# AgentMaker/PAPC

Hardware: AMD Instinct MI355X
Metric: point-clouds/sec (fwd+bwd) PointNet++SSG B=32 N=4096 (higher is better)
Workload: dtype f32

## Files before the change

### include/papc_hip.h

```cpp
#ifndef PAPC_HIP_H
#define PAPC_HIP_H

#include <stddef.h>
#include <stdint.h>

#ifdef __cplusplus
extern "C" {
#endif

#define PAPC_OK 0
#define PAPC_E_INVALID (-1)
#define PAPC_E_UNSUPPORTED (-2)
#define PAPC_E_LAUNCH (-3)

typedef void *papc_stream_t;

int papc_version(void);
#define PAPC_ABI_VERSION 8
int papc_abi_version(void);
int64_t papc_abi_sizeof(const char *struct_name);
const char *papc_last_error_string(void);


int papc_fps_f32(const float *xyz, int64_t sb, int64_t sn, int64_t sc, int B, int N, int npoint,
// ... 337 lines not shown
    const float *x; int32_t Cin, Cout;
    float *dy, *dw, *db, *dgamma, *dbeta; int32_t accumulate;
    int32_t phase;
} papc_head_bwd_job;
int papc_head_chain_fwd_f32(const papc_head_fc_layer *layers, int n_layers, int B, const int64_t *rng_state, int64_t *rng_bump,
                            const int64_t *labels, float *loss, float *dlogits, uint32_t *sync, papc_stream_t stream);
int papc_head_chain_bwd_f32(const papc_head_bwd_job *jobs, int n_jobs, int B, uint32_t *sync, papc_stream_t stream);

int papc_cloud_transform_f32(const float *x, int64_t sb, int64_t sn, int64_t sc, const float *T, int64_t ldt, int B, int N, int C, float *y,
                             papc_stream_t stream);
size_t papc_cloud_transform_bwd_workspace(int B, int N, int C);
int papc_cloud_transform_bwd_f32(const float *x, int64_t sb, int64_t sn, int64_t sc, const float *T, int64_t ldt, const float *dy, int B, int N, int C,
                                 float *dx, int64_t dsb, int64_t dsn, int64_t dsc, int accumulate, float *dT, void *workspace,
                                 size_t workspace_bytes, papc_stream_t stream);

int papc_cloud_concat_conv_parts(int B, int N);
int papc_cloud_concat_conv_f32(const float *x, int64_t ldx, const float *g, const float *w, const float *bias, int B, int N, int Cp, int Cg, int Cout,
                               float *y, float *cvec, float *stats_partial, papc_stream_t stream);
size_t papc_cloud_concat_conv_bwd_workspace(int B, int N, int Cp, int Cg, int Cout);
int papc_cloud_concat_conv_bwd_f32(const float *dz, const float *y, const float *mean, const float *invstd, const float *scale, const float *shift,
                                   const float *c1, const float *c2, const float *x, int64_t ldx, const float *g, const float *w, int B, int N, int Cp,
                                   int Cg, int Cout, float *dx, int64_t ldd, int accumulate, float *dw, float *dbias, float *dg, float *s_out,
                                   void *workspace, size_t workspace_bytes, papc_stream_t stream);

int papc_kdconv_ok(int dim, int Cin, int F);
int papc_kdconv_fwd_f32(const float *x, int64_t ldx, const int32_t *sel, int64_t sel_stride, const float *w, const float *bias, int B, int dim, int Cin,
                        int F, float *out, uint8_t *win, papc_stream_t stream);
size_t papc_kdconv_bwd_workspace(int B, int dim, int Cin, int F);
int papc_kdconv_bwd_f32(const float *gout, const float *out, const uint8_t *win, const float *x, int64_t ldx, const int32_t *sel, int64_t sel_stride,
                        const float *w, int B, int dim, int Cin, int F, float *dx, int64_t ldd, float *dw, float *dbias, int accumulate, void *workspace,
                        size_t workspace_bytes, papc_stream_t stream);

int papc_kdbn_ok(int dim, int Cin, int F);
size_t papc_kdbn_fwd_workspace(int B, int dim, int Cin, int F);
int papc_kdbn_fwd_f32(const float *x, int64_t ldx, const int32_t *sel, int64_t sel_stride, const float *w, const float *bias, const float *gamma,
                      const float *beta, float *running_mean, float *running_var, int B, int dim, int Cin, int F, float eps, float momentum, int training,
                      float *out, uint8_t *win, float *zhat, float *mean, float *tmat, float *stats, void *workspace, size_t workspace_bytes,
                      papc_stream_t stream);
size_t papc_kdbn_bwd_workspace(int B, int dim, int Cin, int F);
int papc_kdbn_bwd_f32(const float *gout, const float *out, const uint8_t *win, const float *zhat, const float *x, int64_t ldx, const int32_t *sel,
                      int64_t sel_stride, const float *w, const float *gamma, const float *mean, const float *tmat, const float *stats, int B, int dim,
                      int Cin, int F, int training, float *dx, int64_t ldd, float *dw, float *dbias, float *dgamma, float *dbeta, int accumulate,
                      void *workspace, size_t workspace_bytes, papc_stream_t stream);

int papc_voxconv_ok(int E);
int papc_voxconv_parts(int B, int E);
int papc_voxconv1_fwd_f32(const float *x, const float *w1, const float *b1, int B, int E, float *y1, float *stats_partial, papc_stream_t stream);
int papc_voxconv2_prep_f32(const float *w2, float *wk, float *wt, papc_stream_t stream);
int papc_voxconv2_pool_fwd_f32(const float *y1, const float *scale, const float *shift, const float *wk, const float *b2, int B, int E, float *out,
                               uint8_t *win, papc_stream_t stream);
int papc_voxconv2_bwd_dx_f32(const float *gout, const uint8_t *win, const float *wt, const float *y1, const float *mean, const float *invstd,
                             const float *scale, const float *shift, int B, int E, float *gp, float *dz, float *red_partial, papc_stream_t stream);
size_t papc_voxconv2_bwd_dw_workspace(int B, int E);
int papc_voxconv2_bwd_dw_f32(const float *gp, const uint8_t *win, const float *y1, const float *scale, const float *shift, int B, int E, float *dw2,
                             float *db2, int accumulate, void *workspace, size_t workspace_bytes, papc_stream_t stream);
size_t papc_voxconv1_bwd_dw_workspace(int B, int E);
int papc_voxconv1_bwd_dw_f32(const float *dz, const float *y1, const float *mean, const float *invstd, const float *scale, const float *c1, const float *c2,
                             const float *x, int B, int E, float *dw1, float *db1, int accumulate, void *workspace, size_t workspace_bytes,
                             papc_stream_t stream);
int papc_leaky_dropout_fwd_f32(const float *x, int64_t n, float slope, float drop_p, int64_t *rng_state, int tag, int bump, float *out, uint8_t *keep,
                               papc_stream_t stream);
int papc_leaky_dropout_bwd_f32(const float *gout, const float *x, const uint8_t *keep, int64_t n, float slope, float drop_p, float *dx,
                               papc_stream_t stream);
int papc_occupancy_grid_f32(const float *points, int B, int N, int E, float *grid, uint32_t *err, papc_stream_t stream);

size_t papc_nms_workspace(int N);
int papc_nms_f32(const float *dets, int N, float nms_overlap_thresh, int32_t *keep, int32_t *num_out, void *workspace,
                 size_t workspace_bytes, papc_stream_t stream);
int papc_rotate_nms_f32(const float *dets, int N, float nms_overlap_thresh, int32_t *keep, int32_t *num_out, void *workspace,
                        size_t workspace_bytes, papc_stream_t stream);
int papc_rotate_iou_f32(const float *boxes, const float *query_boxes, int N, int K, int criterion, float *iou, papc_stream_t stream);
int papc_rbbox_iou_f32(const float *box_corners, const float *qbox_corners, const float *standup_iou, float standup_thresh, int N, int K,
                       float *overlaps, papc_stream_t stream);
int papc_riou_f32(const float *rbboxes, const float *qrbboxes, float standup_thresh, int N, int K, float *overlaps, papc_stream_t stream);

int papc_lingather_parts(int64_t M);
int papc_mlp_compact_ok(int64_t M, int K, int n_layers, const int *couts);
int papc_compact_plan_f32(const int32_t *idx, int G, int K, int32_t *cnt8, int32_t *start, int32_t *rows, int32_t *cidx, int32_t *seg_grp,
                          float *wrow, float *coef, papc_stream_t stream);
int papc_compact_corr_parts(void);
int papc_bn_stats_corr_f32(const float *y, int C, const int32_t *start, const float *coef, int G, float *stats_rows, papc_stream_t stream);
int papc_bn_relu_max_seg_f32(const float *y, int C, const int32_t *start, const float *scale, const float *shift, int G, float *out,
                             int32_t *argmax, float *ysel, papc_stream_t stream);
int papc_lingather_fwd_f32(const float *P, const papc_group_src *grp, int B, const float *w, int ldw, int xcol0, const float *bias, int C,
                           float *y, float *stats_partial, papc_stream_t stream);
int papc_lingather_bwd_f32(const papc_bwd_dy *dy, const papc_group_src *grp, int B, int C, float *G, float *dwx_partial, papc_stream_t stream);
int papc_lingather_bwd_pp_ok(const papc_group_src *grp, int B, int C);
int papc_lingather_bwd_pp_f32(const papc_bwd_dy *dy, const papc_group_src *grp, int B, int C, const float *P, const float *w, int ldw, int xcol0,
                              const float *bias, float *G, float *dwx_partial, papc_stream_t stream);
int papc_lingather_list_parts(int64_t BN);
int papc_lingather_bwd_parts(const papc_group_src *grp, int B, int C);
int papc_lingather_bwd_lists_ok(const papc_group_src *grp, int C);
int papc_point_lists_f32(const papc_group_src *grp, int B, const int32_t *start, int32_t *prange, int32_t *prow, float *pmeta, float *pmom,
                         papc_stream_t stream);

int papc_mlp_bwd_dx_xyz_ok(int64_t M, int Cin, int Cout);
int papc_mlp_bwd_dx_xyz_f32(const papc_bwd_dy *dy, const float *wt, int64_t M, int Cin, int Cout, const float *xc, const float *wf,
                            float *partial, papc_stream_t stream);

int papc_bn_max_prep_f32(const float *gout, const float *ysel, const float *scale, const float *shift, const float *mean,
                         const float *invstd, const float *c1, const float *c2, const float *w, const float *bias, int64_t G, int Co,
                         int Ci, float *psel, float *wcat, float *hbias, float *e_out, float *q_out, papc_stream_t stream);
int papc_mlp_bwd_dx_max_f32(const float *psel, const int32_t *argmax, int K, const float *x, int64_t ldx, const float *bn_scale,
                            const float *bn_shift, const float *wcat, const float *hbias, int64_t M, int Cin, int Cout, float *dx,
                            const papc_bwd_red *next_red, papc_stream_t stream);

int papc_mlp_max_nostore_ok(int64_t M, int Cin, int Cout, int K);
int64_t papc_mlp_bwd_dw_max_ws_floats(int64_t M, int Cin, int Cout);
int papc_mlp_bwd_dw_max_f32(const float *psel, const int32_t *argmax, int K, const float *x, const float *bn_scale, const float *bn_shift,
                            const float *w, const float *e, const float *scale, const float *c1, int64_t M, int Cin, int Cout,
                            float *workspace, float *dw, int accumulate, papc_stream_t stream);

int papc_mlp_xyz_ok(int64_t M, int C1, int C2);
int papc_xyz_parts(int64_t M);
int papc_xyz_bwd_parts(int64_t M);
int papc_xyz_group_f32(const papc_group_src *grp, int B, float *xc, double *gram_partial, papc_stream_t stream);
int papc_xyz_gram_fold_f32(const double *gram_partial, int parts, double *gram, papc_stream_t stream);
int papc_xyz_l1_finalize_f32(const double *gram_partial, int parts, int64_t M, const float *w, int ldw, int xcol0, const float *bias,
                             const float *gamma, const float *beta, float eps, float momentum, int C, float *mean, float *invstd, float *scale,
                             float *shift, float *running_mean, float *running_var, float *wf, double *gram, papc_stream_t stream);
int papc_xyz_l1_bwd_f32(const float *dz, const float *xc, const float *wf, int64_t M, int C, float *partial, papc_stream_t stream);
int papc_xyz_l1_bwd_finalize_f32(const float *partial, int parts, int64_t M, int C, const double *gram, const float *w, int ldw, int xcol0,
                                 const float *bias, const float *mean, const float *invstd, const float *scale, float *dgamma, float *dbeta,
                                 float *dw, int accumulate, papc_stream_t stream);

size_t papc_pg_planes_bytes(int64_t R, int64_t K);

typedef struct papc_pg_wjob {
    const float *src;
    int64_t row_stride, col_stride;
    int R, K;
    void *planes;
} papc_pg_wjob;
int papc_pg_prep_weights_f32(const papc_pg_wjob *jobs, int count, papc_stream_t stream);

#define PAPC_PG_PLAIN 0
#define PAPC_PG_CONCAT 1
#define PAPC_PG_BNRELU 2
#define PAPC_PG_DY_DENSE 3
#define PAPC_PG_DY_MAX 4
typedef struct papc_pg_prep {
    int mode;
    int64_t M; int C;
    const float *x; int64_t ldx;
    const float *xyz; int64_t sb, sn, sc; const float *feats; int N, D, xyz_first;
    const float *dz;
    const float *gout, *ysel; const int32_t *argmax; int K;
    const float *stats; int parts;
    const float *gamma, *beta; float eps, momentum; float *running_mean, *running_var;
    float *mean, *invstd, *scale, *shift;
    const float *red; int red_parts;
    float *dgamma, *dbeta; int accumulate;
    void *planes, *planes_t;
} papc_pg_prep;
int papc_pg_prep_rows_f32(const papc_pg_prep *args, papc_stream_t stream);

#define PAPC_PG_STORE 0
#define PAPC_PG_FWD 1
#define PAPC_PG_FWD_GMAX 2
#define PAPC_PG_RED 3
typedef struct papc_pg_gemm {
    int epi;
    const void *a, *b;
    int R1, R2, K;
    float *c; int64_t ldc;
    int split; int64_t split_stride;
// ... 77 lines not shown
```

### papc_amd/_lib.py

```python
import ctypes
import os

_HERE = os.path.dirname(os.path.abspath(__file__))
LIB_PATH = os.environ.get("PAPC_LIB") or os.path.join(_HERE, "libpapc_hip.so")

ABI_VERSION = 8

c_p = ctypes.c_void_p
c_i = ctypes.c_int
c_l = ctypes.c_int64
c_f = ctypes.c_float


class PapcError(RuntimeError):
    pass


class GroupSrc(ctypes.Structure):
    _fields_ = [("xyz", c_p), ("sb", c_l), ("sn", c_l), ("sc", c_l), ("new_xyz", c_p), ("feats", c_p),
                ("idx", c_p), ("N", c_i), ("S", c_i), ("K", c_i), ("D", c_i), ("xyz_first", c_i),
                ("cidx", c_p), ("seg_grp", c_p), ("rows_dev", c_p), ("wstat", c_p), ("plists", c_p)]


class PointLists(ctypes.Structure):
    _fields_ = [("prange", c_p), ("prow", c_p), ("pmeta", c_p), ("compact", c_i), ("pmom", c_p)]


class BwdDy(ctypes.Structure):
    _fields_ = [("dz_mode", c_i), ("dz", c_p), ("gout", c_p), ("argmax", c_p), ("K", c_i), ("y", c_p),
                ("mean", c_p), ("invstd", c_p), ("scale", c_p), ("shift", c_p), ("c1", c_p), ("c2", c_p),
                ("wrow", c_p), ("seg_grp", c_p), ("rows_dev", c_p), ("psel", c_p)]

    def set_bn(self, y, cst, c12):
        self.y = ptr(y)
        self.mean, self.invstd, self.scale, self.shift = cst_ptrs(cst)
        self.c1, self.c2 = c12.data_ptr(), c12.data_ptr() + 4 * c12.stride(0)


class GroupMax(ctypes.Structure):
    _fields_ = [("gmax", c_p), ("gmin", c_p), ("amax", c_p), ("amin", c_p), ("K", c_i), ("sign_src", c_p)]


class BwdRed(ctypes.Structure):
    _fields_ = [("y", c_p), ("mean", c_p), ("invstd", c_p), ("scale", c_p), ("shift", c_p), ("red_partial", c_p), ("store_masked", c_i)]


class CopyJob(ctypes.Structure):
    _fields_ = [("src", ctypes.c_void_p), ("dst", ctypes.c_void_p), ("B", ctypes.c_int32), ("R", ctypes.c_int32), ("C", ctypes.c_int32),
                ("sb", ctypes.c_int64), ("sr", ctypes.c_int64), ("sc", ctypes.c_int64), ("db", ctypes.c_int64), ("dr", ctypes.c_int64),
                ("dc", ctypes.c_int64)]


class ReduceJob(ctypes.Structure):
    _fields_ = [("partial", c_p), ("n_chunks", ctypes.c_int32), ("accumulate", ctypes.c_int32), ("ld", c_l), ("n1", c_l), ("n2", c_l),
                ("out1", c_p), ("out2", c_p)]


class ScatterDst(ctypes.Structure):
    _fields_ = [("grad_feats", c_p), ("idx", c_p), ("N", c_i), ("S", c_i), ("K", c_i), ("D", c_i), ("col0", c_i)]


SIGNATURES = {
    "papc_version": (c_i, []),
    "papc_abi_version": (c_i, []),
    "papc_abi_sizeof": (c_l, [ctypes.c_char_p]),
    "papc_last_error_string": (ctypes.c_char_p, []),
    "papc_fps_f32": (c_i, [c_p, c_l, c_l, c_l, c_i, c_i, c_i, c_p, c_f, c_p, c_p, c_p]),
    "papc_ball_query_f32": (c_i, [c_p, c_l, c_l, c_l, c_p, c_i, c_i, c_i, c_i, c_p, c_p, c_p, c_i, c_p]),
    "papc_square_distance_f32": (c_i, [c_p, c_p, c_i, c_i, c_i, c_p, c_p]),
    "papc_index_points_f32": (c_i, [c_p, c_p, c_i, c_i, c_i, c_i, c_i, c_p, c_p]),
    "papc_index_points_bwd_f32": (c_i, [c_p, c_p, c_i, c_i, c_i, c_i, c_i, c_p, c_p]),
    "papc_group_points_f32": (c_i, [c_p, c_l, c_l, c_l, c_p, c_p, c_p, c_i, c_i, c_i, c_i, c_i, c_i, c_p, c_p]),
    "papc_group_points_bwd_f32": (c_i, [c_p, c_p, c_i, c_i, c_i, c_i, c_i, c_i, c_p, c_p, c_p, c_p]),
    "papc_three_nn_f32": (c_i, [c_p, c_l, c_l, c_l, c_p, c_l, c_l, c_l, c_i, c_i, c_i, c_p, c_p, c_p, c_p]),
    "papc_three_interpolate_f32": (c_i, [c_p, c_p, c_p, c_i, c_i, c_i, c_i, c_p, c_p]),
    "papc_three_interpolate_bwd_f32": (c_i, [c_p, c_p, c_p, c_i, c_i, c_i, c_i, c_p, c_p]),
    "papc_three_interpolate_bwd_first3_f32": (c_i, [c_p, c_p, c_i, c_i, c_i, c_i, c_p, c_p]),
    "papc_mlp_gemm_parts": (c_i, [c_l]),
    "papc_mlp_gemm_gmax_ok": (c_i, [c_l, c_i, c_i]),
    "papc_mlp_gemm_f32": (c_i, [c_i, c_p, c_l, c_p, c_p, c_p, c_p, c_p, c_l, c_i, c_i, c_p, c_p, c_p, c_p]),
    "papc_mlp_gemm_rows_f32": (c_i, [c_i, c_p, c_l, c_p, c_p, c_p, c_p, c_p, c_l, c_i, c_i, c_p, c_p, c_p, c_p, c_p]),
    "papc_mlp_gemm_rows_w_f32": (c_i, [c_i, c_p, c_l, c_p, c_p, c_p, c_p, c_p, c_l, c_i, c_i, c_p, c_p, c_p, c_p, c_p, c_p]),
    "papc_sa_mlp_plan": (c_i, [c_p, c_p, c_p]),
    "papc_sa_mlp_fwd": (c_i, [c_p, c_p, c_p]),
    "papc_sa_mlp_bwd": (c_i, [c_p, c_p, c_p, c_p]),
    "papc_pfn_workspace": (c_i, [c_p, c_p, c_p]),
    "papc_pfn_fwd": (c_i, [c_p, c_p, c_p]),
    "papc_pfn_bwd": (c_i, [c_p, c_p, c_p, c_p, c_p, c_p, c_i, c_p]),
    "papc_compact_plan_f32": (c_i, [c_p, c_i, c_i, c_p, c_p, c_p, c_p, c_p, c_p, c_p, c_p]),
    "papc_compact_corr_parts": (c_i, []),
    "papc_mlp_compact_ok": (c_i, [c_l, c_i, c_i, c_p]),
    "papc_bn_stats_corr_f32": (c_i, [c_p, c_i, c_p, c_p, c_i, c_p, c_p]),
    "papc_bn_relu_max_seg_f32": (c_i, [c_p, c_i, c_p, c_p, c_p, c_i, c_p, c_p, c_p, c_p]),
    "papc_bn_select_max_f32": (c_i, [c_p, c_p, c_p, c_p, c_p, c_p, c_l, c_i, c_p, c_p, c_p]),
    "papc_bn_finalize_f32": (c_i, [c_p, c_i, c_l, c_i, c_p, c_p, c_f, c_f, c_p, c_p, c_p, c_p, c_p, c_p, c_p]),
    "papc_bn_relu_max_f32": (c_i, [c_p, c_p, c_p, c_l, c_i, c_i, c_p, c_p, c_p]),
    "papc_bn_relu_f32": (c_i, [c_p, c_p, c_p, c_l, c_i, c_p, c_p]),
    "papc_bn_bwd_reduce_max_f32": (c_i, [c_p, c_p, c_i, c_p, c_p, c_p, c_p, c_l, c_i, c_i, c_p, c_p, c_p]),
    "papc_bn_bwd_reduce_f32": (c_i, [c_i, c_p, c_p, c_p, c_i, c_p, c_p, c_p, c_p, c_p, c_l, c_i, c_i, c_p, c_p]),
    "papc_bn_bwd_finalize_f32": (c_i, [c_p, c_i, c_l, c_i, c_p, c_p, c_p, c_p, c_i, c_p]),
    "papc_bn_eval_consts_f32": (c_i, [c_p, c_p, c_p, c_p, c_f, c_i, c_p, c_p, c_p, c_p, c_p]),
    "papc_group_max_bwd_f32": (c_i, [c_p, c_p, c_l, c_i, c_i, c_p, c_p]),
    "papc_mlp_bwd_dx_f32": (c_i, [c_p, c_p, c_l, c_i, c_i, c_p, c_p, c_p, c_p]),
    "papc_mlp_bwd_dw_f32": (c_i, [c_p, c_i, c_p, c_l, c_p, c_p, c_p, c_l, c_i, c_i, c_i, c_p, c_p, c_l, c_p]),
    "papc_reduce_partials2_f32": (c_i, [c_p, c_i, c_l, c_l, c_p, c_l, c_p, c_i, c_p]),
    "papc_reduce_partials_batch_f32": (c_i, [c_p, c_i, c_p]),
    "papc_fold_jobs_f32": (c_i, [c_p, c_i, c_p]),
    "papc_mlp_bwd_dw_chunk_hint": (c_i, [c_l, c_i, c_i, c_i, c_i, c_i]),
    "papc_reduce_partials_f32": (c_i, [c_p, c_i, c_l, c_p, c_i, c_p]),
    "papc_pfn_decorate_f32": (c_i, [c_p, c_p, c_p, c_i, c_i, c_f, c_f, c_f, c_f, c_i, c_p, c_p]),
    "papc_pfn_decorate_nf_f32": (c_i, [c_p, c_i, c_p, c_p, c_i, c_i, c_f, c_f, c_f, c_f, c_i, c_p, c_p]),
    "papc_pfn_stats_f32": (c_i, [c_p, c_p, c_p, c_i, c_i, c_f, c_f, c_f, c_f, c_p, c_i, c_p, c_p, c_p]),
    "papc_pfn_apply_f32": (c_i, [c_p, c_p, c_p, c_i, c_i, c_f, c_f, c_f, c_f, c_p, c_i, c_p, c_p, c_p, c_p, c_p]),
    "papc_pfn_num_blocks": (c_i, [c_i]),
    "papc_pfn_bwd_reduce_f32": (c_i, [c_p, c_p, c_p, c_i, c_i, c_f, c_f, c_f, c_f, c_p, c_i, c_p, c_p, c_p, c_p, c_p, c_p, c_p, c_p]),
    "papc_pfn_bwd_dw_f32": (c_i, [c_p, c_p, c_p, c_i, c_i, c_f, c_f, c_f, c_f, c_p, c_i, c_p, c_p, c_p, c_p, c_p, c_p, c_p, c_p, c_p, c_p]),
    "papc_pfn_gram_blocks": (c_i, [c_i]),
    "papc_pfn_gram_f32": (c_i, [c_p, c_p, c_p, c_i, c_i, c_f, c_f, c_f, c_f, c_p, c_p]),
    "papc_pfn_gram_finalize_f32": (c_i, [c_p, c_i, c_l, c_p, c_i, c_p, c_p, c_f, c_f, c_p, c_p, c_p, c_p, c_p, c_p, c_p, c_p]),
    "papc_pfn_bwd_sparse_f32": (c_i, [c_p, c_p, c_p, c_i, c_i, c_f, c_f, c_f, c_f, c_p, c_i, c_p, c_p, c_p, c_p, c_p, c_p, c_p, c_p]),
    "papc_pfn_bwd_finalize_f32": (c_i, [c_p, c_l, c_p, c_i, c_p, c_p, c_p, c_p, c_p, c_p, c_p, c_i, c_p]),
    "papc_points_to_voxel_workspace": (ctypes.c_size_t, [c_i]),
    "papc_points_to_voxel_f32": (c_i, [c_p, c_i, c_i, c_p, c_p, c_i, c_i, c_i, c_p, c_p, c_p, c_p, c_p, ctypes.c_size_t, c_p]),
    "papc_pillar_scatter_f32": (c_i, [c_p, c_p, c_i, c_i, c_i, c_i, c_i, c_p, c_p, c_p]),
    "papc_pillar_scatter_bwd_f32": (c_i, [c_p, c_p, c_p, c_i, c_i, c_i, c_i, c_i, c_p, c_p]),
    "papc_head_fc_f32": (c_i, [c_p, c_p, c_p, c_p, c_p, c_i, c_i, c_i, c_i, c_f, c_f, c_p, c_p, c_p, c_f, c_p, c_i, c_p, c_p, c_p, c_p,
                               c_p, c_p, c_p]),
    "papc_head_bwd_f32": (c_i, [c_p, c_p, c_i, c_p, c_p, c_p, c_p, c_p, c_f, c_i, c_p, c_i, c_i, c_i, c_p, c_p, c_p, c_p, c_p, c_i, c_p]),
    "papc_softmax_xent_f32": (c_i, [c_p, c_p, c_i, c_i, c_p, c_p, c_p]),
    "papc_head_chain_fwd_f32": (c_i, [c_p, c_i, c_i, c_p, c_p, c_p, c_p, c_p, c_p, c_p]),
    "papc_head_chain_bwd_f32": (c_i, [c_p, c_i, c_i, c_p, c_p]),
    "papc_cloud_transform_f32": (c_i, [c_p, c_l, c_l, c_l, c_p, c_l, c_i, c_i, c_i, c_p, c_p]),
    "papc_cloud_transform_bwd_workspace": (ctypes.c_size_t, [c_i, c_i, c_i]),
    "papc_cloud_transform_bwd_f32": (c_i, [c_p, c_l, c_l, c_l, c_p, c_l, c_p, c_i, c_i, c_i, c_p, c_l, c_l, c_l, c_i, c_p, c_p, ctypes.c_size_t, c_p]),
    "papc_cloud_concat_conv_parts": (c_i, [c_i, c_i]),
    "papc_cloud_concat_conv_f32": (c_i, [c_p, c_l, c_p, c_p, c_p, c_i, c_i, c_i, c_i, c_i, c_p, c_p, c_p, c_p]),
    "papc_cloud_concat_conv_bwd_workspace": (ctypes.c_size_t, [c_i, c_i, c_i, c_i, c_i]),
    "papc_cloud_concat_conv_bwd_f32": (c_i, [c_p, c_p, c_p, c_p, c_p, c_p, c_p, c_p, c_p, c_l, c_p, c_p, c_i, c_i, c_i, c_i, c_i, c_p, c_l, c_i, c_p, c_p,
                                             c_p, c_p, c_p, ctypes.c_size_t, c_p]),
    "papc_kdconv_ok": (c_i, [c_i, c_i, c_i]),
    "papc_kdconv_fwd_f32": (c_i, [c_p, c_l, c_p, c_l, c_p, c_p, c_i, c_i, c_i, c_i, c_p, c_p, c_p]),
    "papc_kdconv_bwd_workspace": (ctypes.c_size_t, [c_i, c_i, c_i, c_i]),
    "papc_kdconv_bwd_f32": (c_i, [c_p, c_p, c_p, c_p, c_l, c_p, c_l, c_p, c_i, c_i, c_i, c_i, c_p, c_l, c_p, c_p, c_i, c_p, ctypes.c_size_t, c_p]),
    "papc_kdbn_ok": (c_i, [c_i, c_i, c_i]),
    "papc_kdbn_fwd_workspace": (ctypes.c_size_t, [c_i, c_i, c_i, c_i]),
    "papc_kdbn_fwd_f32": (c_i, [c_p, c_l, c_p, c_l, c_p, c_p, c_p, c_p, c_p, c_p, c_i, c_i, c_i, c_i, c_f, c_f, c_i, c_p, c_p, c_p, c_p, c_p, c_p, c_p,
                                ctypes.c_size_t, c_p]),
    "papc_kdbn_bwd_workspace": (ctypes.c_size_t, [c_i, c_i, c_i, c_i]),
    "papc_kdbn_bwd_f32": (c_i, [c_p, c_p, c_p, c_p, c_p, c_l, c_p, c_l, c_p, c_p, c_p, c_p, c_p, c_i, c_i, c_i, c_i, c_i, c_p, c_l, c_p, c_p, c_p, c_p, c_i,
                                c_p, ctypes.c_size_t, c_p]),
    "papc_voxconv_ok": (c_i, [c_i]),
    "papc_voxconv_parts": (c_i, [c_i, c_i]),
    "papc_voxconv1_fwd_f32": (c_i, [c_p, c_p, c_p, c_i, c_i, c_p, c_p, c_p]),
    "papc_voxconv2_prep_f32": (c_i, [c_p, c_p, c_p, c_p]),
    "papc_voxconv2_pool_fwd_f32": (c_i, [c_p, c_p, c_p, c_p, c_p, c_i, c_i, c_p, c_p, c_p]),
    "papc_voxconv2_bwd_dx_f32": (c_i, [c_p] * 8 + [c_i, c_i, c_p, c_p, c_p, c_p]),
    "papc_voxconv2_bwd_dw_workspace": (ctypes.c_size_t, [c_i, c_i]),
    "papc_voxconv2_bwd_dw_f32": (c_i, [c_p, c_p, c_p, c_p, c_p, c_i, c_i, c_p, c_p, c_i, c_p, ctypes.c_size_t, c_p]),
    "papc_voxconv1_bwd_dw_workspace": (ctypes.c_size_t, [c_i, c_i]),
    "papc_voxconv1_bwd_dw_f32": (c_i, [c_p] * 8 + [c_i, c_i, c_p, c_p, c_i, c_p, ctypes.c_size_t, c_p]),
    "papc_leaky_dropout_fwd_f32": (c_i, [c_p, c_l, c_f, c_f, c_p, c_i, c_i, c_p, c_p, c_p]),
    "papc_leaky_dropout_bwd_f32": (c_i, [c_p, c_p, c_p, c_l, c_f, c_f, c_p, c_p]),
    "papc_occupancy_grid_f32": (c_i, [c_p, c_i, c_i, c_i, c_p, c_p, c_p]),
    "papc_nms_workspace": (ctypes.c_size_t, [c_i]),
    "papc_nms_f32": (c_i, [c_p, c_i, c_f, c_p, c_p, c_p, ctypes.c_size_t, c_p]),
    "papc_lingather_parts": (c_i, [c_l]),
    "papc_lingather_fwd_f32": (c_i, [c_p, c_p, c_i, c_p, c_i, c_i, c_p, c_i, c_p, c_p, c_p]),
    "papc_lingather_bwd_f32": (c_i, [c_p, c_p, c_i, c_i, c_p, c_p, c_p]),
    "papc_lingather_bwd_pp_f32": (c_i, [c_p, c_p, c_i, c_i, c_p, c_p, c_i, c_i, c_p, c_p, c_p, c_p]),
    "papc_lingather_list_parts": (c_i, [c_l]),
    "papc_lingather_bwd_parts": (c_i, [c_p, c_i, c_i]),
    "papc_lingather_bwd_lists_ok": (c_i, [c_p, c_i]),
    "papc_point_lists_f32": (c_i, [c_p, c_i, c_p, c_p, c_p, c_p, c_p, c_p]),
    "papc_lingather_bwd_pp_ok": (c_i, [c_p, c_i, c_i]),
    "papc_bn_max_prep_f32": (c_i, [c_p] * 10 + [c_l, c_i, c_i] + [c_p] * 6),
    "papc_mlp_max_nostore_ok": (c_i, [c_l, c_i, c_i, c_i]),
# ... 146 lines not shown
```

### papc_amd/csrc/bn_ops.hip

```cpp
#include "common.h"

namespace papc {

template <int V> struct Vec;
template <> struct Vec<4> {
    float4 v;
    __device__ static Vec load(const float *p) { Vec r; r.v = *reinterpret_cast<const float4 *>(p); return r; }
    __device__ void store(float *p) const { *reinterpret_cast<float4 *>(p) = v; }
    __device__ float &operator[](int i) { return (&v.x)[i]; }
    __device__ float operator[](int i) const { return (&v.x)[i]; }
};
template <> struct Vec<1> {
    float v;
    __device__ static Vec load(const float *p) { Vec r; r.v = *p; return r; }
    __device__ void store(float *p) const { *p = v; }
    __device__ float &operator[](int) { return v; }
    __device__ float operator[](int) const { return v; }
};

template <int D>
__device__ __forceinline__ void sum_partial_rows_d(const float *__restrict__ part, int n_tiles, int C, int c, int tl, double &s1, double &s2)
{
    for (int t0 = tl; t0 < n_tiles; t0 += 64 * D) {
        float a[D], b[D];
#pragma unroll
        for (int j = 0; j < D; ++j) {
            const int t = t0 + 64 * j;
            const int64_t o = (int64_t)(t < n_tiles ? t : t0) * 2 * C + c;
            a[j] = part[o];
            b[j] = part[o + C];
        }
#pragma unroll
        for (int j = 0; j < D; ++j) {
            if (t0 + 64 * j < n_tiles) { s1 += (double)a[j]; s2 += (double)b[j]; }
        }
    }
}
__device__ __forceinline__ void sum_partial_rows(const float *__restrict__ part, int n_tiles, int C, int c, int tl, double &s1, double &s2)
{
    if (n_tiles > 512) sum_partial_rows_d<16>(part, n_tiles, C, c, tl, s1, s2);
    else sum_partial_rows_d<8>(part, n_tiles, C, c, tl, s1, s2);
}

__device__ __forceinline__ double lane_get(double v, int l)
{
    const int lo = __builtin_amdgcn_readlane(__double2loint(v), l), hi = __builtin_amdgcn_readlane(__double2hiint(v), l);
    return __hiloint2double(hi, lo);
}
__device__ __forceinline__ void fold_part_lanes(double &s1, double &s2)
{
    s1 += __shfl_xor(s1, 1); s2 += __shfl_xor(s2, 1);
    s1 += __shfl_xor(s1, 2); s2 += __shfl_xor(s2, 2);
    double t1 = 0.0, t2 = 0.0;
#pragma unroll
    for (int w = 0; w < 16; ++w) { t1 += lane_get(s1, 4 * w); t2 += lane_get(s2, 4 * w); }
    s1 = t1; s2 = t2;
}

__global__ __launch_bounds__(64) void bn_finalize_kernel(const float *__restrict__ part, int n_tiles, int64_t M, int C,
                                                        const float *__restrict__ gamma, const float *__restrict__ beta,
                                                        float eps, float momentum, float *mean, float *invstd, float *scale,
                                                        float *shift, float *rmean, float *rvar)
{
    const int c = blockIdx.x, tl = threadIdx.x;
    const float gam = gamma ? gamma[c] : 1.f, bet = beta ? beta[c] : 0.f;
    const float rm0 = rmean ? rmean[c] : 0.f, rv0 = rvar ? rvar[c] : 0.f;
    double s1 = 0.0, s2 = 0.0;
    sum_partial_rows(part, n_tiles, C, c, tl, s1, s2);
    fold_part_lanes(s1, s2);
    if (tl == 0) {
        const double mu = s1 / (double)M;
        double var = s2 / (double)M - mu * mu;
        if (var < 0.0) var = 0.0;
        const double is = 1.0 / sqrt(var + (double)eps);
        const double sc = (double)gam * is;
        mean[c] = (float)mu;
        invstd[c] = (float)is;
        scale[c] = (float)sc;
        shift[c] = (float)((double)bet - mu * sc);
        if (rmean) rmean[c] = momentum * rm0 + (1.f - momentum) * (float)mu;
        if (rvar) rvar[c] = momentum * rv0 + (1.f - momentum) * (float)var;
    }
}

template <int V>
__global__ __launch_bounds__(256) void bn_relu_max_kernel(const float *__restrict__ y, const float *__restrict__ scale,
                                                          const float *__restrict__ shift, int64_t G, int K, int C,
                                                          float *__restrict__ out, int32_t *__restrict__ argmax)
{
    const int CV = C / V;
    const int64_t total = G * CV;
    for (int64_t e = (int64_t)blockIdx.x * blockDim.x + threadIdx.x; e < total; e += (int64_t)gridDim.x * blockDim.x) {
        const int64_t g = e / CV;
        const int c = (int)(e - g * CV) * V;
        const Vec<V> sc = Vec<V>::load(scale + c), sh = Vec<V>::load(shift + c);
        Vec<V> best;
        int bi[V];
#pragma unroll
        for (int i = 0; i < V; ++i) { best[i] = -1.0f; bi[i] = 0; }
        const float *yp = y + (g * K) * (int64_t)C + c;
        for (int k = 0; k < K; ++k) {
            const Vec<V> v = Vec<V>::load(yp + (int64_t)k * C);
#pragma unroll
            for (int i = 0; i < V; ++i) {
                const float z = relu_np(fmaf(sc[i], v[i], sh[i]));
                if (z > best[i] || z != z) { best[i] = z; bi[i] = k; }
            }
        }
        best.store(out + g * C + c);
        if (argmax) {
#pragma unroll
            for (int i = 0; i < V; ++i) argmax[g * C + c + i] = bi[i];
        }
    }
}

__global__ __launch_bounds__(256) void bn_select_max_kernel(float *__restrict__ gmax, const float *__restrict__ gmin,
                                                            const int32_t *__restrict__ amax, const int32_t *__restrict__ amin,
                                                            const float *__restrict__ scale, const float *__restrict__ shift,
                                                            int64_t total, int C, float *__restrict__ out, int32_t *__restrict__ argmax)
{
    for (int64_t e = (int64_t)blockIdx.x * blockDim.x + threadIdx.x; e < total; e += (int64_t)gridDim.x * blockDim.x) {
        const int c = (int)(e % C);
        const float sc = scale[c], sh = shift[c];
        const bool up = sc >= 0.f;
        const float sel = up ? gmax[e] : gmin[e];
        out[e] = relu_np(fmaf(sc, sel, sh));
        gmax[e] = sel;
        if (argmax) argmax[e] = up ? amax[e] : amin[e];
    }
}

template <int V>
__global__ __launch_bounds__(256) void bn_relu_kernel(const float *__restrict__ y, const float *__restrict__ scale,
                                                      const float *__restrict__ shift, int64_t M, int C, float *__restrict__ z)
{
    const int CV = C / V;
    const int64_t total = M * CV;
    for (int64_t e = (int64_t)blockIdx.x * blockDim.x + threadIdx.x; e < total; e += (int64_t)gridDim.x * blockDim.x) {
        const int c = (int)(e % CV) * V;
        const Vec<V> sc = Vec<V>::load(scale + c), sh = Vec<V>::load(shift + c);
        Vec<V> v = Vec<V>::load(y + e * V);
#pragma unroll
        for (int i = 0; i < V; ++i) v[i] = fmaxf(fmaf(sc[i], v[i], sh[i]), 0.f);
        v.store(z + e * V);
    }
}

template <int V, bool MAXMODE>
__global__ __launch_bounds__(256) void bn_bwd_reduce_kernel(const float *__restrict__ dz, const float *__restrict__ gout,
                                                            const int32_t *__restrict__ argmax, int K,
                                                            const float *__restrict__ y, const float *__restrict__ mean,
                                                            const float *__restrict__ invstd, const float *__restrict__ scale,
                                                            const float *__restrict__ shift, int64_t M, int C,
                                                            float *__restrict__ part, float *__restrict__ psel_out = nullptr)
{
    __shared__ float red[2][256 * 4];
    const int CV = C / V;
    const int CG = CV < 256 ? CV : 256;
    const int RL = 256 / CG;
    const int cgi = threadIdx.x % CG, rl = threadIdx.x / CG;
    const int64_t units = MAXMODE ? M / K : M;
    const int64_t per = (units + gridDim.x - 1) / gridDim.x;
    const int64_t u0 = (int64_t)blockIdx.x * per, u1 = min(units, u0 + per);

// ... 296 lines not shown

__global__ __launch_bounds__(256) void bn_max_psel_kernel(const float *__restrict__ gout, const float *__restrict__ ysel,
                                                          const float *__restrict__ scale, const float *__restrict__ shift, int64_t total,
                                                          int C, float *__restrict__ psel)
{
    for (int64_t e = (int64_t)blockIdx.x * blockDim.x + threadIdx.x; e < total; e += (int64_t)gridDim.x * blockDim.x) {
        const int c = (int)(e % C);
        const float sc = scale[c];
        psel[e] = fmaf(sc, ysel[e], shift[c]) > 0.f ? sc * gout[e] : 0.f;
    }
}

__global__ __launch_bounds__(256) void bn_max_wcat_kernel(const float *__restrict__ w, const float *__restrict__ bias,
                                                          const float *__restrict__ scale, const float *__restrict__ mean,
                                                          const float *__restrict__ invstd, const float *__restrict__ c1,
                                                          const float *__restrict__ c2, int Co, int Ci, float *__restrict__ wcat,
                                                          float *__restrict__ hbias, float *__restrict__ e_out, float *__restrict__ q_out)
{
    extern __shared__ float sm[];
    float *ewn = sm;
    double *red = reinterpret_cast<double *>(sm + ((Co + 1) & ~1));
    const int n = blockIdx.x, tid = threadIdx.x;
    double hacc = 0.0;
    for (int c = tid; c < Co; c += 256) {
        const float s = scale[c];
        const float e = s * c2[c] * invstd[c];
        const float q = e * (mean[c] - (bias ? bias[c] : 0.f)) - s * c1[c];
        const float wv = w[(int64_t)c * Ci + n];
        ewn[c] = e * wv;
        hacc += (double)q * (double)wv;
        wcat[(int64_t)n * (Co + Ci) + c] = wv;
        if (n == 0) { e_out[c] = e; q_out[c] = q; }
    }
    red[tid] = hacc;
    __syncthreads();
    for (int st = 128; st > 0; st >>= 1) {
        if (tid < st) red[tid] += red[tid + st];
        __syncthreads();
    }
    if (tid == 0) hbias[n] = (float)red[0];
    for (int j = tid; j < Ci; j += 256) {
        double g = 0.0;
        for (int c = 0; c < Co; ++c) g += (double)ewn[c] * (double)w[(int64_t)c * Ci + j];
        wcat[(int64_t)n * (Co + Ci) + Co + j] = (float)(-g);
    }
}

struct TransposeBatch {
    const float *src[8];
    float *dst[8];
    int rows[8], cols[8];
    int ld[8], copy[8];
};

__global__ __launch_bounds__(256) void transpose_batch_kernel(TransposeBatch t)
{
    __shared__ float tile[32][33];
    const int m = blockIdx.y;
    const int rows = t.rows[m], cols = t.cols[m];
    const int tiles_c = (cols + 31) >> 5, tiles = ((rows + 31) >> 5) * tiles_c;
    const float *__restrict__ src = t.src[m];
    float *__restrict__ dst = t.dst[m];
    const int tx = threadIdx.x & 31, ty = threadIdx.x >> 5;
    for (int tl = blockIdx.x; tl < tiles; tl += gridDim.x) {
        const int r0 = (tl / tiles_c) * 32, c0 = (tl % tiles_c) * 32;
#pragma unroll
        for (int i = 0; i < 4; ++i) {
            const int r = r0 + ty + 8 * i, c = c0 + tx;
            const float v = (r < rows && c < cols) ? src[(int64_t)r * t.ld[m] + c] : 0.f;
            tile[ty + 8 * i][tx] = v;
            if (t.copy[m] && r < rows && c < cols) dst[(int64_t)r * cols + c] = v;
        }
        if (t.copy[m]) continue;
        __syncthreads();
#pragma unroll
        for (int i = 0; i < 4; ++i) {
            const int c = c0 + ty + 8 * i, r = r0 + tx;
            if (r < rows && c < cols) dst[(int64_t)c * rows + r] = tile[tx][ty + 8 * i];
        }
        __syncthreads();
    }
}

}


using namespace papc;

extern "C" {

int papc_bn_finalize_f32(const float *stats_partial, int n_tiles, int64_t M, int C, const float *gamma,
                         const float *beta, float eps, float momentum, float *mean, float *invstd,
                         float *scale, float *shift, float *running_mean, float *running_var,
                         papc_stream_t stream)
{
    PAPC_REQUIRE(stats_partial && mean && invstd && scale && shift, PAPC_E_INVALID, "papc_bn_finalize_f32: null pointer");
    PAPC_REQUIRE(n_tiles >= 1 && M >= 1 && C >= 1, PAPC_E_INVALID, "papc_bn_finalize_f32: bad sizes");
    hipStream_t st = as_stream(stream);
    ProfScope prof(PAPC_K_MISC, st);
    hipLaunchKernelGGL(bn_finalize_kernel, dim3((unsigned)C), dim3(64), 0, st, stats_partial, n_tiles, M, C, gamma,
                       beta, eps, momentum, mean, invstd, scale, shift, running_mean, running_var);
    return check_launch("papc_bn_finalize_f32");
}

int papc_bn_relu_max_f32(const float *y, const float *scale, const float *shift, int64_t G, int K, int C,
                         float *out, int32_t *argmax, papc_stream_t stream)
{
    PAPC_REQUIRE(y && scale && shift && out, PAPC_E_INVALID, "papc_bn_relu_max_f32: null pointer");
    PAPC_REQUIRE(G >= 1 && K >= 1 && C >= 1, PAPC_E_INVALID, "papc_bn_relu_max_f32: bad sizes");
    hipStream_t st = as_stream(stream);
    ProfScope prof(PAPC_K_BN_RELU_MAX, st);
    const bool v4 = (C % 4 == 0) && aligned16(y) && aligned16(scale) && aligned16(shift) && aligned16(out);
    if (v4 && K >= 256 && G * (C / 4) < 65536 && G <= 65535) {
        hipLaunchKernelGGL(bn_relu_max_split_kernel, dim3((unsigned)G, (unsigned)cdiv(C, 256)), dim3(1024), 0, st, y, scale, shift, G, K, C, out, argmax);
        return check_launch("papc_bn_relu_max_f32");
    }
    if (v4) hipLaunchKernelGGL(bn_relu_max_kernel<4>, dim3(ew_grid(G * (C / 4))), dim3(256), 0, st, y, scale, shift, G, K, C, out, argmax);
    else hipLaunchKernelGGL(bn_relu_max_kernel<1>, dim3(ew_grid(G * C)), dim3(256), 0, st, y, scale, shift, G, K, C, out, argmax);
    return check_launch("papc_bn_relu_max_f32");
}

int papc_bn_select_max_f32(float *gmax, const float *gmin, const int32_t *amax, const int32_t *amin,
                           const float *scale, const float *shift, int64_t G, int C, float *out, int32_t *argmax,
                           papc_stream_t stream)
{
    PAPC_REQUIRE(gmax && gmin && amax && amin && scale && shift && out, PAPC_E_INVALID, "papc_bn_select_max_f32: null pointer");
    PAPC_REQUIRE(G >= 1 && C >= 1, PAPC_E_INVALID, "papc_bn_select_max_f32: bad sizes");
    hipStream_t st = as_stream(stream);
    ProfScope prof(PAPC_K_BN_RELU_MAX, st);
    hipLaunchKernelGGL(bn_select_max_kernel, dim3(ew_grid(G * C)), dim3(256), 0, st, gmax, gmin, amax, amin, scale, shift, G * C, C, out, argmax);
    return check_launch("papc_bn_select_max_f32");
}

int papc_bn_relu_f32(const float *y, const float *scale, const float *shift, int64_t M, int C, float *z, papc_stream_t stream)
{
    PAPC_REQUIRE(y && scale && shift && z, PAPC_E_INVALID, "papc_bn_relu_f32: null pointer");
    PAPC_REQUIRE(M >= 1 && C >= 1, PAPC_E_INVALID, "papc_bn_relu_f32: bad sizes");
    hipStream_t st = as_stream(stream);
    ProfScope prof(PAPC_K_MISC, st);
    const bool v4 = (C % 4 == 0) && aligned16(y) && aligned16(scale) && aligned16(shift) && aligned16(z);
    if (v4) hipLaunchKernelGGL(bn_relu_kernel<4>, dim3(ew_grid(M * (C / 4))), dim3(256), 0, st, y, scale, shift, M, C, z);
    else hipLaunchKernelGGL(bn_relu_kernel<1>, dim3(ew_grid(M * C)), dim3(256), 0, st, y, scale, shift, M, C, z);
    return check_launch("papc_bn_relu_f32");
}

int papc_bn_bwd_reduce_f32(int dz_mode, const float *dz, const float *gout, const int32_t *argmax, int K,
                           const float *y, const float *mean, const float *invstd, const float *scale,
                           const float *shift, int64_t M, int C, int n_parts, float *red_partial, papc_stream_t stream)
{
    PAPC_REQUIRE(mean && invstd && scale && shift && red_partial, PAPC_E_INVALID, "papc_bn_bwd_reduce_f32: null pointer");
    PAPC_REQUIRE(y || (dz_mode != PAPC_DZ_DENSE && dz), PAPC_E_INVALID, "papc_bn_bwd_reduce_f32: y may be NULL only in MAX mode with dz = ysel");
    PAPC_REQUIRE(M >= 1 && C >= 1 && n_parts >= 1, PAPC_E_INVALID, "papc_bn_bwd_reduce_f32: bad sizes");
    hipStream_t st = as_stream(stream);
    ProfScope prof(PAPC_K_BWD_REDUCE, st);
    if (dz_mode == PAPC_DZ_DENSE) {
        PAPC_REQUIRE(dz, PAPC_E_INVALID, "papc_bn_bwd_reduce_f32: DENSE needs dz");
        const bool v4 = (C % 4 == 0) && aligned16(dz) && aligned16(y) && aligned16(mean) && aligned16(invstd) && aligned16(scale) && aligned16(shift);
        if (v4) hipLaunchKernelGGL((bn_bwd_reduce_kernel<4, false>), dim3(n_parts), dim3(256), 0, st, dz, gout, argmax, K, y, mean, invstd, scale, shift, M, C, red_partial);
        else hipLaunchKernelGGL((bn_bwd_reduce_kernel<1, false>), dim3(n_parts), dim3(256), 0, st, dz, gout, argmax, K, y, mean, invstd, scale, shift, M, C, red_partial);
    } else {
        PAPC_REQUIRE(gout && argmax && K >= 1 && M % K == 0, PAPC_E_INVALID, "papc_bn_bwd_reduce_f32: MAX needs gout/argmax and K | M");
        const bool v4 = (C % 4 == 0) && aligned16(gout) && (!dz || aligned16(dz)) && aligned16(mean) && aligned16(invstd) && aligned16(scale) && aligned16(shift);
        if (v4) hipLaunchKernelGGL((bn_bwd_reduce_kernel<4, true>), dim3(n_parts), dim3(256), 0, st, dz, gout, argmax, K, y, mean, invstd, scale, shift, M, C, red_partial);
        else hipLaunchKernelGGL((bn_bwd_reduce_kernel<1, true>), dim3(n_parts), dim3(256), 0, st, dz, gout, argmax, K, y, mean, invstd, scale, shift, M, C, red_partial);
    }
    return check_launch("papc_bn_bwd_reduce_f32");
// ... 224 lines not shown
```

### papc_amd/csrc/capi.hip

```cpp
#include <stdarg.h>
#include <string.h>

#include <mutex>
#include <vector>

#include "common.h"

#define GEMM_PARTS_DEFAULT 768

namespace papc {

static thread_local char g_err[512] = "";

void set_error(const char *fmt, ...)
{
    va_list ap;
    va_start(ap, fmt);
    vsnprintf(g_err, sizeof(g_err), fmt, ap);
    va_end(ap);
}

int check_launch(const char *what)
{
    hipError_t e = hipGetLastError();
    if (e != hipSuccess) {
        set_error("%s: %s", what, hipGetErrorString(e));
        return PAPC_E_LAUNCH;
    }
    return PAPC_OK;
}

struct KnobDef { const char *name; int def, lo, hi; };
static const KnobDef g_knob_defs[KNOB_COUNT] = {
    {"PAPC_LG_PARTS", 2048, 1, 8192},
    {"PAPC_DW_F32", 0, 0, 1},
    {"PAPC_DW_DBG", 0, 0, 1},
    {"PAPC_DW_XYZ", 1, 0, 1},
    {"PAPC_PARTS", GEMM_PARTS_DEFAULT, 1, 1024},
    {"PAPC_GEMM_F32", 0, 0, 1},
    {"PAPC_GEMM_WAVES", 0, 0, 8},
    {"PAPC_MAXCAT_WAVES", 8, 4, 8},
    {"PAPC_GEMM_WS", 0, 0, 3},
    {"PAPC_GEMM_OCC", 0, 0, 1},
    {"PAPC_GEMM_DBG", 0, 0, 1},
    {"PAPC_GEMM_KB", 0, 0, 2},
    {"PAPC_GEMM_MINWG", 192, 1, 4096},
    {"PAPC_GEMM_TL", 0, 0, 1},
    {"PAPC_FPS_THREADS", 0, 0, 1024},
    {"PAPC_FPS_THREADS_SMALL", 0, 0, 1024},
    {"PAPC_STREAM", 1, 0, 1},
    {"PAPC_STREAM_MINTILES", 2048, 1, 1 << 30},
    {"PAPC_STREAM_CK", 0, 0, 8},
    {"PAPC_STREAM_ASM", 1, 0, 1},
    {"PAPC_PFN_MFMA", 1, 0, 1},
    {"PAPC_DW_RS64", 1, 0, 1},
    {"PAPC_DW_ROWS", 1, 0, 1},
    {"PAPC_DW_ROWS_BLOCKS", 4, 1, 16},
    {"PAPC_DW_ROWSX", 1, 0, 1},
    {"PAPC_PG_DBG", 0, 0, 15},
    {"PAPC_PG_NB", 0, 0, 2},
    {"PAPC_PG_NS", 0, 0, 3},
    {"PAPC_STREAM_MAXCAT", 1, 0, 1},
    {"PAPC_MAX_NOSTORE", 1, 0, 1},
    {"PAPC_PFN_FUSED_TAILS", 1, 0, 1},
    {"PAPC_STREAM_NW12", 1, 0, 1},
    {"PAPC_LG_LISTS", 1, 0, 1},
    {"PAPC_FOLD_WAVES", 16, 8, 16},
    {"PAPC_LGL_VARIANT", 0, 0, 3},
    {"PAPC_LG_PP", 1, 0, 1},
    {"PAPC_PG_GROUP", 1, 0, 1},
    {"PAPC_PG_PIPE", 1, 0, 1},
};
static int g_knobs[KNOB_COUNT];
static int knob_parse(int id, const char *e)
{
    const KnobDef &d = g_knob_defs[id];
    if (!e || !*e) return d.def;
    const int v = atoi(e);
    return (v < d.lo || v > d.hi) ? d.def : v;
}
static const bool g_knobs_loaded = [] {
    for (int i = 0; i < KNOB_COUNT; ++i) g_knobs[i] = knob_parse(i, getenv(g_knob_defs[i].name));
    return true;
}();
int knob(int id) { return g_knobs[id]; }

struct ProfState {
    std::mutex mu;
    unsigned mask = 0;
    std::vector<std::pair<hipEvent_t, hipEvent_t>> pending[PAPC_K_COUNT];
    std::vector<hipEvent_t> pool;
    double total_ms[PAPC_K_COUNT] = {0};
    int64_t launches[PAPC_K_COUNT] = {0};
};
static ProfState g_prof;

static hipEvent_t prof_get_event()
{
    if (!g_prof.pool.empty()) {
        hipEvent_t e = g_prof.pool.back();
        g_prof.pool.pop_back();
        return e;
    }
    hipEvent_t e;
    if (hipEventCreate(&e) != hipSuccess) return nullptr;
    return e;
}

ProfScope::ProfScope(int k, hipStream_t s) : kernel(k), stream(s), on(false), e0(nullptr)
{
    if (!(g_prof.mask & (1u << k))) return;
    std::lock_guard<std::mutex> lk(g_prof.mu);
    e0 = prof_get_event();
    if (!e0) return;
    on = hipEventRecord(e0, stream) == hipSuccess;
}

ProfScope::~ProfScope()
{
    if (!on) return;
    std::lock_guard<std::mutex> lk(g_prof.mu);
    hipEvent_t e1 = prof_get_event();
    if (!e1) return;
    if (hipEventRecord(e1, stream) == hipSuccess) g_prof.pending[kernel].push_back({e0, e1});
}

static void prof_drain(int k)
{
    for (auto &pr : g_prof.pending[k]) {
        float ms = 0.f;
        if (hipEventSynchronize(pr.second) == hipSuccess && hipEventElapsedTime(&ms, pr.first, pr.second) == hipSuccess) {
            g_prof.total_ms[k] += ms;
            g_prof.launches[k] += 1;
        }
        g_prof.pool.push_back(pr.first);
        g_prof.pool.push_back(pr.second);
    }
    g_prof.pending[k].clear();
}

}

extern "C" {

int papc_version(void) { return 600;  }

int papc_abi_version(void) { return PAPC_ABI_VERSION; }

int64_t papc_abi_sizeof(const char *struct_name)
{
    if (!struct_name) return -1;
#define PAPC_SIZEOF(T) if (strcmp(struct_name, #T) == 0) return (int64_t)sizeof(T);
    PAPC_SIZEOF(papc_group_src)
    PAPC_SIZEOF(papc_point_lists)
// ... 81 lines not shown
```

### papc_amd/csrc/common.h

```cpp
#pragma once
#include <hip/hip_runtime.h>
#include <stdint.h>
#include <stdio.h>
#include <stdlib.h>
#include <string.h>
#include <algorithm>

#include "papc_hip.h"

namespace papc {

void set_error(const char *fmt, ...);
int check_launch(const char *what);

#define PAPC_REQUIRE(cond, code, ...)      \
    do {                                   \
        if (!(cond)) {                     \
            papc::set_error(__VA_ARGS__);  \
            return (code);                 \
        }                                  \
    } while (0)

enum Knob {
    KNOB_LG_PARTS, KNOB_DW_F32, KNOB_DW_DBG, KNOB_DW_XYZ, KNOB_PARTS, KNOB_GEMM_F32, KNOB_GEMM_WAVES, KNOB_MAXCAT_WAVES,
    KNOB_GEMM_WS, KNOB_GEMM_OCC, KNOB_GEMM_DBG, KNOB_GEMM_KB, KNOB_GEMM_MINWG, KNOB_GEMM_TL, KNOB_FPS_THREADS,
    KNOB_FPS_THREADS_SMALL, KNOB_STREAM, KNOB_STREAM_MINTILES, KNOB_STREAM_CK, KNOB_STREAM_ASM, KNOB_PFN_MFMA, KNOB_DW_RS64, KNOB_DW_ROWS, KNOB_DW_ROWS_BLOCKS, KNOB_DW_ROWSX, KNOB_PG_DBG, KNOB_PG_NB, KNOB_PG_NS, KNOB_STREAM_MAXCAT, KNOB_MAX_NOSTORE, KNOB_PFN_FUSED_TAILS, KNOB_STREAM_NW12, KNOB_LG_LISTS, KNOB_FOLD_WAVES, KNOB_LGL_VARIANT, KNOB_LG_PP, KNOB_PG_GROUP, KNOB_PG_PIPE, KNOB_COUNT
};
int knob(int id);

struct ProfScope {
    int kernel;
    hipStream_t stream;
    bool on;
    hipEvent_t e0;
    ProfScope(int kernel, hipStream_t stream);
    ~ProfScope();
};

static inline hipStream_t as_stream(papc_stream_t s) { return reinterpret_cast<hipStream_t>(s); }

static inline int64_t cdiv(int64_t a, int64_t b) { return (a + b - 1) / b; }
static inline bool aligned16(const void *p) { return (reinterpret_cast<uintptr_t>(p) & 15) == 0; }

#define PAPC_DPP(v, ctrl, rmask) __builtin_amdgcn_update_dpp((int)(v), (int)(v), (ctrl), (rmask), 0xF, false)

__device__ __forceinline__ float wave_sum_f32_to_lane63(float v)
{
    float t;
    t = __int_as_float(PAPC_DPP(__float_as_int(v), 0xB1, 0xF));  v += t;
    t = __int_as_float(PAPC_DPP(__float_as_int(v), 0x4E, 0xF));  v += t;
    t = __int_as_float(PAPC_DPP(__float_as_int(v), 0x124, 0xF)); v += t;
    t = __int_as_float(PAPC_DPP(__float_as_int(v), 0x128, 0xF)); v += t;
    t = __int_as_float(__builtin_amdgcn_update_dpp(0, __float_as_int(v), 0x142, 0xA, 0xF, false)); v += t;
    t = __int_as_float(__builtin_amdgcn_update_dpp(0, __float_as_int(v), 0x143, 0xC, 0xF, false)); v += t;
    return v;
}

__device__ __forceinline__ float half_sum_f32(float v)
{
    float t;
    t = __int_as_float(PAPC_DPP(__float_as_int(v), 0xB1, 0xF));  v += t;
    t = __int_as_float(PAPC_DPP(__float_as_int(v), 0x4E, 0xF));  v += t;
    t = __int_as_float(PAPC_DPP(__float_as_int(v), 0x124, 0xF)); v += t;
    t = __int_as_float(PAPC_DPP(__float_as_int(v), 0x128, 0xF)); v += t;
    t = __int_as_float(__builtin_amdgcn_update_dpp(0, __float_as_int(v), 0x142, 0xA, 0xF, false)); v += t;
    return v;
}

__device__ __forceinline__ float readlane63_f32(float v)
{
    return __int_as_float(__builtin_amdgcn_readlane(__float_as_int(v), 63));
}


#define PAPC_DPPF(v, ctrl, rmask) __int_as_float(__builtin_amdgcn_update_dpp(__float_as_int(v), __float_as_int(v), (ctrl), (rmask), 0xF, false))
#define PAPC_DPPU(v, ctrl, rmask) ((unsigned)__builtin_amdgcn_update_dpp((int)(v), (int)(v), (ctrl), (rmask), 0xF, false))

__device__ __forceinline__ float row_max_f32(float v)
{
    v = fmaxf(v, PAPC_DPPF(v, 0xB1, 0xF));
    v = fmaxf(v, PAPC_DPPF(v, 0x4E, 0xF));
    v = fmaxf(v, PAPC_DPPF(v, 0x124, 0xF));
    v = fmaxf(v, PAPC_DPPF(v, 0x128, 0xF));
    return v;
}
__device__ __forceinline__ unsigned row_min_u32(unsigned v)
{
    unsigned t;
    t = PAPC_DPPU(v, 0xB1, 0xF);  v = t < v ? t : v;
    t = PAPC_DPPU(v, 0x4E, 0xF);  v = t < v ? t : v;
    t = PAPC_DPPU(v, 0x124, 0xF); v = t < v ? t : v;
    t = PAPC_DPPU(v, 0x128, 0xF); v = t < v ? t : v;
    return v;
}
__device__ __forceinline__ float wave_max_f32_to_lane63(float v)
{
    v = row_max_f32(v);
    v = fmaxf(v, PAPC_DPPF(v, 0x142, 0xA));
    v = fmaxf(v, PAPC_DPPF(v, 0x143, 0xC));
    return v;
}
__device__ __forceinline__ unsigned wave_min_u32_to_lane63(unsigned v)
{
    unsigned t;
    v = row_min_u32(v);
    t = PAPC_DPPU(v, 0x142, 0xA); v = t < v ? t : v;
    t = PAPC_DPPU(v, 0x143, 0xC); v = t < v ? t : v;
    return v;
}
// ... 47 lines not shown
```

### papc_amd/csrc/compact.hip

```cpp
#include "common.h"

namespace papc {

__global__ __launch_bounds__(256) void compact_count_kernel(const int32_t *__restrict__ idx, int G, int K, int32_t *__restrict__ cnt8)
{
    const int g = blockIdx.x * 4 + (threadIdx.x >> 6), lane = threadIdx.x & 63;
    if (g >= G) return;
    const int32_t *row = idx + (int64_t)g * K;
    const int32_t first = row[0];
    int n = 0;
    for (int k = lane; k < K; k += 64) n += (k > 0 && row[k] != first) ? 1 : 0;
#pragma unroll
    for (int o = 32; o > 0; o >>= 1) n += __shfl_xor(n, o);
    if (lane == 0) cnt8[g] = (n + 1 + 7) & ~7;
}

__global__ __launch_bounds__(1024) void compact_scan_kernel(const int32_t *__restrict__ cnt8, int G, int32_t *__restrict__ start,
                                                            int32_t *__restrict__ rows)
{
    __shared__ int part[1024];
    const int tid = threadIdx.x;
    const int per = (G + 1023) / 1024;
    const int g0 = tid * per, g1 = min(G, g0 + per);
    int s = 0;
// ... 60 lines not shown
                }
#pragma unroll
                for (int u = 0; u < U; ++u) {
                    s1.x = fmaf(cf[u], v[u].x, s1.x); s1.y = fmaf(cf[u], v[u].y, s1.y); s1.z = fmaf(cf[u], v[u].z, s1.z); s1.w = fmaf(cf[u], v[u].w, s1.w);
                    s2.x = fmaf(cf[u] * v[u].x, v[u].x, s2.x); s2.y = fmaf(cf[u] * v[u].y, v[u].y, s2.y);
                    s2.z = fmaf(cf[u] * v[u].z, v[u].z, s2.z); s2.w = fmaf(cf[u] * v[u].w, v[u].w, s2.w);
                }
            }
        }
        red[0][threadIdx.x] = s1; red[1][threadIdx.x] = s2;
        __syncthreads();
        const int cqn = CQ < 256 ? CQ : 256;
        if ((int)threadIdx.x < cqn && c0 + (int)threadIdx.x < CQ) {
            float4 t1 = make_float4(0.f, 0.f, 0.f, 0.f), t2 = t1;
            for (int l = 0; l < RL; ++l) {
                const float4 a = red[0][l * cqn + threadIdx.x], b = red[1][l * cqn + threadIdx.x];
                t1.x += a.x; t1.y += a.y; t1.z += a.z; t1.w += a.w;
                t2.x += b.x; t2.y += b.y; t2.z += b.z; t2.w += b.w;
            }
            *reinterpret_cast<float4 *>(out + ((int64_t)r * 2 + 0) * C + 4 * (c0 + threadIdx.x)) = t1;
            *reinterpret_cast<float4 *>(out + ((int64_t)r * 2 + 1) * C + 4 * (c0 + threadIdx.x)) = t2;
        }
        __syncthreads();
    }
}

__global__ __launch_bounds__(256) void seg_max_kernel(const float *__restrict__ y, int C, const int32_t *__restrict__ start,
                                                      const float *__restrict__ scale, const float *__restrict__ shift, int G,
                                                      float *__restrict__ out, int32_t *__restrict__ argmax, float *__restrict__ ysel)
{
    const int CQ = C >> 2;
    const int64_t e = (int64_t)blockIdx.x * 256 + threadIdx.x;
    if (e >= (int64_t)G * CQ) return;
    const int g = (int)(e / CQ), c = (int)(e - (int64_t)g * CQ) * 4;
    const int r0 = start[g], r1 = start[g + 1];
    const float4 sc = *reinterpret_cast<const float4 *>(scale + c), sh = *reinterpret_cast<const float4 *>(shift + c);
    const float s4[4] = {sc.x, sc.y, sc.z, sc.w}, h4[4] = {sh.x, sh.y, sh.z, sh.w};
    int flip[4];
#pragma unroll
    for (int i = 0; i < 4; ++i) flip[i] = s4[i] >= 0.f ? 0 : (int)0x80000000u;
    float mx[4] = {-INFINITY, -INFINITY, -INFINITY, -INFINITY};
    int ix[4] = {r0, r0, r0, r0};
    const float *p = y + (int64_t)r0 * C + c;
    int r = r0;
    for (; r + 4 <= r1; r += 4) {
        float4 v[4];
#pragma unroll
        for (int u = 0; u < 4; ++u) v[u] = *reinterpret_cast<const float4 *>(p + (int64_t)u * C);
#pragma unroll
        for (int u = 0; u < 4; ++u) {
            const float a[4] = {v[u].x, v[u].y, v[u].z, v[u].w};
#pragma unroll
            for (int i = 0; i < 4; ++i) {
                const float k = __int_as_float(__float_as_int(a[i]) ^ flip[i]);
                if (k > mx[i]) { mx[i] = k; ix[i] = r + u; }
            }
        }
        p += (int64_t)4 * C;
    }
    for (; r < r1; ++r) {
        const float4 v = *reinterpret_cast<const float4 *>(p);
        const float a[4] = {v.x, v.y, v.z, v.w};
#pragma unroll
        for (int i = 0; i < 4; ++i) {
            const float k = __int_as_float(__float_as_int(a[i]) ^ flip[i]);
            if (k > mx[i]) { mx[i] = k; ix[i] = r; }
        }
        p += C;
    }
    float o[4], ys[4];
    int am[4];
#pragma unroll
    for (int i = 0; i < 4; ++i) {
        ys[i] = __int_as_float(__float_as_int(mx[i]) ^ flip[i]);
        am[i] = ix[i];
        o[i] = relu_np(fmaf(s4[i], ys[i], h4[i]));
    }
    const int64_t q = (int64_t)g * C + c;
    *reinterpret_cast<float4 *>(out + q) = make_float4(o[0], o[1], o[2], o[3]);
    *reinterpret_cast<int4 *>(argmax + q) = make_int4(am[0], am[1], am[2], am[3]);
    *reinterpret_cast<float4 *>(ysel + q) = make_float4(ys[0], ys[1], ys[2], ys[3]);
}

}

using namespace papc;

extern "C" {

int papc_compact_plan_f32(const int32_t *idx, int G, int K, int32_t *cnt8, int32_t *start, int32_t *rows, int32_t *cidx, int32_t *seg_grp,
                          float *wrow, float *coef, papc_stream_t stream)
{
    PAPC_REQUIRE(idx && cnt8 && start && rows && cidx && seg_grp && wrow && coef, PAPC_E_INVALID, "papc_compact_plan_f32: null pointer");
    PAPC_REQUIRE(G >= 1 && K >= 8 && K % 8 == 0, PAPC_E_UNSUPPORTED, "papc_compact_plan_f32: G=%d, nsample=%d must be a multiple of 8", G, K);
    PAPC_REQUIRE((int64_t)G * K < (1ll << 31), PAPC_E_UNSUPPORTED, "papc_compact_plan_f32: >= 2^31 rows");
    hipStream_t st = as_stream(stream);
    ProfScope prof(PAPC_K_GROUP, st);
    const unsigned nb = (unsigned)cdiv(G, 4);
    hipLaunchKernelGGL(compact_count_kernel, dim3(nb), dim3(256), 0, st, idx, G, K, cnt8);
    hipLaunchKernelGGL(compact_scan_kernel, dim3(1), dim3(1024), 0, st, cnt8, G, start, rows);
    hipLaunchKernelGGL(compact_fill_kernel, dim3(nb), dim3(256), 0, st, idx, G, K, start, rows, cidx, seg_grp, wrow, coef);
    return check_launch("papc_compact_plan_f32");
}

int papc_compact_corr_parts(void) { return 64; }

int papc_bn_stats_corr_f32(const float *y, int C, const int32_t *start, const float *coef, int G, float *stats_rows, papc_stream_t stream)
{
    PAPC_REQUIRE(y && start && coef && stats_rows, PAPC_E_INVALID, "papc_bn_stats_corr_f32: null pointer");
    PAPC_REQUIRE(G >= 1 && C >= 4 && C % 4 == 0 && aligned16(y) && aligned16(stats_rows), PAPC_E_INVALID, "papc_bn_stats_corr_f32: C %% 4 == 0 and 16-byte aligned rows");
    hipStream_t st = as_stream(stream);
    ProfScope prof(PAPC_K_MISC, st);
    hipLaunchKernelGGL(bn_stats_corr_kernel, dim3((unsigned)papc_compact_corr_parts()), dim3(256), 0, st, y, C, start, coef, G, stats_rows);
    return check_launch("papc_bn_stats_corr_f32");
}

int papc_bn_relu_max_seg_f32(const float *y, int C, const int32_t *start, const float *scale, const float *shift, int G, float *out,
                             int32_t *argmax, float *ysel, papc_stream_t stream)
{
    PAPC_REQUIRE(y && start && scale && shift && out && argmax && ysel, PAPC_E_INVALID, "papc_bn_relu_max_seg_f32: null pointer");
    PAPC_REQUIRE(G >= 1 && C >= 4 && C % 4 == 0, PAPC_E_UNSUPPORTED, "papc_bn_relu_max_seg_f32: C=%d must be a multiple of 4", C);
    PAPC_REQUIRE(aligned16(y) && aligned16(scale) && aligned16(shift) && aligned16(out) && aligned16(argmax) && aligned16(ysel), PAPC_E_INVALID,
                 "papc_bn_relu_max_seg_f32: 16-byte alignment");
    hipStream_t st = as_stream(stream);
    ProfScope prof(PAPC_K_BN_RELU_MAX, st);
    hipLaunchKernelGGL(seg_max_kernel, dim3((unsigned)cdiv((int64_t)G * (C / 4), 256)), dim3(256), 0, st, y, C, start, scale, shift, G, out, argmax, ysel);
    return check_launch("papc_bn_relu_max_seg_f32");
}

}
```

### papc_amd/csrc/mlp_gemm.h

```cpp
#pragma once
#include "mlp_loaders.h"

namespace papc {

enum { EPI_STORE = 0, EPI_SCATTER = 1, EPI_STORE_RED = 2, EPI_STORE_GMAX = 3, EPI_GMAX = 4, EPI_XYZ_RED = 5 };

struct RedSrc {
    const float *y; const float *mean, *invstd, *scale, *shift;
    int masked;
};

struct ScatterDst {
    float *gf; const int32_t *idx; int N, S, K, D;
    FastDiv divSK, divK;
};

struct GmaxDst {
    float *gmax, *gmin; int32_t *amax, *amin; int K;
    const float *sgn;
};

struct GemmArgs {
    ASrc a;
    const float *w; int64_t ldw;
    int wmap;
    int nmap;
    const float *bias;
    int64_t M; int Kin; int Nout;
    float *y; int64_t ldy;
    float *stats;
    int parts;
    ScatterDst sc;
    RedSrc rd;
    GmaxDst gm;
    const int32_t *rows_dev;
    const float *wstat;
    unsigned long long *dbg;
    int tl;
};

constexpr int GEMM_MAX_PARTS = 768;

int stream_gemm_try(const GemmArgs &p, int amode, int epi, bool vec, hipStream_t st);

}
```

### papc_amd/csrc/mlp_gemm.hip

```cpp
#include "mlp_gemm.h"
#include <mutex>
#include <unordered_map>

namespace papc {

constexpr int LDT = 36;
constexpr int BK = 32;

template <bool VEC, bool WMAP, bool NMAP>
__device__ __forceinline__ float4 fetch_w4(const GemmArgs &p, int n, int k)
{
    const int nn = n < p.Nout ? n : 0;
    const int nrow = NMAP ? gk(p.a.g, nn) : nn;
    const float *wr = p.w + (int64_t)nrow * p.ldw;
    float4 v;
    if (WMAP) {
        v.x = wr[k < p.Kin ? gk(p.a.g, k) : 0];
        v.y = wr[k + 1 < p.Kin ? gk(p.a.g, k + 1) : 0];
        v.z = wr[k + 2 < p.Kin ? gk(p.a.g, k + 2) : 0];
        v.w = wr[k + 3 < p.Kin ? gk(p.a.g, k + 3) : 0];
    } else if (VEC) {
        v = ld4(wr + (k < p.Kin ? k : 0));
    } else {
        v.x = wr[k < p.Kin ? k : 0];
// ... 805 lines not shown
    g.idx = s->idx; g.N = s->N; g.S = s->S; g.K = s->K; g.D = s->D; g.xyz_first = s->xyz_first;
    g.divK = make_fastdiv((uint32_t)s->K);
    g.divS = make_fastdiv((uint32_t)s->S);
}

void fill_dy(DySrc &d, const papc_bwd_dy *s)
{
    d.dz = s->dz; d.gout = s->gout; d.argmax = s->argmax; d.K = s->K > 0 ? s->K : 1; d.y = s->y; d.mean = s->mean;
    d.invstd = s->invstd; d.scale = s->scale; d.shift = s->shift; d.c1 = s->c1; d.c2 = s->c2;
    d.divK = make_fastdiv((uint32_t)d.K);
    d.C = 0;
    d.wrow = s->wrow; d.seg_grp = s->seg_grp; d.rows_dev = s->rows_dev; d.psel = s->psel;
}

int check_dy(const papc_bwd_dy *dy, int64_t M, int C, bool *vec, const char *who)
{
    PAPC_REQUIRE(dy && dy->y && dy->mean && dy->invstd && dy->scale && dy->shift && dy->c1 && dy->c2, PAPC_E_INVALID,
                 "%s: null pointer in dy", who);
    const bool cst = aligned16(dy->mean) && aligned16(dy->invstd) && aligned16(dy->scale) && aligned16(dy->shift) &&
                     aligned16(dy->c1) && aligned16(dy->c2);
    if (dy->dz_mode == PAPC_DZ_DENSE) {
        PAPC_REQUIRE(dy->dz, PAPC_E_INVALID, "%s: DENSE needs dz", who);
        *vec = cst && aligned16(dy->dz) && aligned16(dy->y) && (C % 4 == 0);
    } else if (dy->dz_mode == PAPC_DZ_MAX) {
        PAPC_REQUIRE(dy->gout && dy->argmax && dy->K >= 1 && M % dy->K == 0, PAPC_E_INVALID, "%s: MAX needs gout/argmax and K | M", who);
        *vec = cst && aligned16(dy->gout) && aligned16(dy->argmax) && aligned16(dy->y) && (C % 4 == 0);
    } else {
        set_error("%s: bad dz_mode %d", who, dy->dz_mode);
        return PAPC_E_INVALID;
    }
    return PAPC_OK;
}

int fill_asrc(ASrc &a, int a_mode, const float *x, int64_t ldx, const papc_group_src *grp, const float *sc,
              const float *sh, int Cin, const char *who)
{
    memset(&a, 0, sizeof(a));
    if (a_mode == A_PLAIN || a_mode == A_BNRELU) {
        PAPC_REQUIRE(x && ldx >= Cin, PAPC_E_INVALID, "%s: x null or ldx < Cin", who);
        PAPC_REQUIRE(a_mode == A_PLAIN || (sc && sh), PAPC_E_INVALID, "%s: BNRELU needs bn_scale/bn_shift", who);
        a.x = x; a.ldx = ldx; a.sc = sc; a.sh = sh;
        a.vec = aligned16(x) && (ldx % 4 == 0) && (Cin % 4 == 0) && (a_mode == A_PLAIN || (aligned16(sc) && aligned16(sh)));
    } else if (a_mode == A_XYZ) {
        PAPC_REQUIRE(x && ldx == 4 && sc, PAPC_E_INVALID, "%s: XYZ needs xc [M, 4] (ldx = 4) and the folded first layer wf [Cin, 4] as bn_scale", who);
        a.x = x; a.ldx = 4; a.sc = sc; a.sh = nullptr;
        a.vec = aligned16(x) && aligned16(sc) && Cin % 4 == 0;
    } else if (a_mode == A_GROUP) {
        PAPC_REQUIRE(grp && grp->xyz && grp->new_xyz, PAPC_E_INVALID, "%s: GROUP needs grp->xyz/new_xyz", who);
        PAPC_REQUIRE(grp->D == 0 || grp->feats, PAPC_E_INVALID, "%s: GROUP D=%d but feats null", who, grp->D);
        PAPC_REQUIRE(Cin == grp->D + 3, PAPC_E_INVALID, "%s: GROUP Cin=%d != D+3=%d", who, Cin, grp->D + 3);
        PAPC_REQUIRE(grp->N >= 1 && grp->S >= 1 && grp->K >= 1, PAPC_E_INVALID, "%s: GROUP bad N/S/K", who);
        fill_group(a.g, grp);
        a.vec = (grp->D == 0) || (aligned16(grp->feats) && (grp->D % 4 == 0));
    } else {
        set_error("%s: bad a_mode %d", who, a_mode);
        return PAPC_E_INVALID;
    }
    return PAPC_OK;
}

}

using namespace papc;

extern "C" {

int papc_mlp_gemm_parts(int64_t M) { return gemm_parts(M); }

int papc_mlp_gemm_gmax_ok(int64_t M, int Cout, int K)
{
    if (!(K == 32 || K == 64 || K == 128) || M % 128 != 0 || Cout <= 32 || Cout % 32 != 0) return 0;
    if (K == 128 && !(Cout == 64 || Cout % 128 == 0)) return 0;
    return gemm_col_tile(gemm_parts(M), Cout) != 32;
}

int papc_mlp_gemm_f32(int a_mode, const float *x, int64_t ldx, const papc_group_src *grp,
                      const float *bn_scale, const float *bn_shift, const float *w, const float *bias,
                      int64_t M, int Cin, int Cout, float *y, float *stats_partial, const papc_group_max *gmax,
                      papc_stream_t stream)
{
    return papc_mlp_gemm_rows_f32(a_mode, x, ldx, grp, bn_scale, bn_shift, w, bias, M, Cin, Cout, y, stats_partial, gmax, nullptr, stream);
}

int papc_mlp_gemm_rows_w_f32(int a_mode, const float *x, int64_t ldx, const papc_group_src *grp,
                           const float *bn_scale, const float *bn_shift, const float *w, const float *bias,
                           int64_t M, int Cin, int Cout, float *y, float *stats_partial, const papc_group_max *gmax,
                           const int32_t *rows_dev, const float *wrow, papc_stream_t stream)
{
    PAPC_REQUIRE(w && (y || gmax), PAPC_E_INVALID, "papc_mlp_gemm_f32: null w/y");
    PAPC_REQUIRE(!rows_dev || (!gmax && (a_mode == A_PLAIN || a_mode == A_BNRELU)), PAPC_E_UNSUPPORTED,
                 "papc_mlp_gemm_rows_f32: a device-side row count goes with plain / BN+ReLU rows and no fused group max");
    PAPC_REQUIRE(M >= 1 && Cin >= 1 && Cout >= 1, PAPC_E_INVALID, "papc_mlp_gemm_f32: M=%lld Cin=%d Cout=%d", (long long)M, Cin, Cout);
    PAPC_REQUIRE(M < (1ll << 31), PAPC_E_UNSUPPORTED, "papc_mlp_gemm_f32: M=%lld >= 2^31 rows", (long long)M);
    GemmArgs p;
    memset(&p, 0, sizeof(p));
    int rc = fill_asrc(p.a, a_mode, x, ldx, grp, bn_scale, bn_shift, Cin, "papc_mlp_gemm_f32");
    if (rc) return rc;
    p.w = w; p.ldw = Cin; p.bias = bias; p.M = M; p.Kin = Cin; p.Nout = Cout; p.y = y; p.ldy = Cout; p.stats = stats_partial;
    p.rows_dev = rows_dev;
    p.wstat = rows_dev ? wrow : nullptr;
    p.wmap = (a_mode == A_GROUP) ? 1 : 0;
    const bool vec = p.a.vec && (p.wmap || (aligned16(w) && Cin % 4 == 0));
    hipStream_t st = as_stream(stream);
    ProfScope prof(PAPC_K_MLP_GEMM, st);
    PAPC_REQUIRE(!(gmax && a_mode == A_XYZ), PAPC_E_UNSUPPORTED, "papc_mlp_gemm_f32: PAPC_A_XYZ has no fused group-max flavour");
    if (gmax) {
        PAPC_REQUIRE(gmax->gmax && gmax->gmin && gmax->amax && gmax->amin, PAPC_E_INVALID, "papc_mlp_gemm_f32: null pointer in gmax");
        PAPC_REQUIRE(papc_mlp_gemm_gmax_ok(M, Cout, gmax->K), PAPC_E_UNSUPPORTED,
                     "papc_mlp_gemm_f32: fused group max needs K in {32,64,128}, M %% 128 == 0, Cout > 32 (got K=%d M=%lld Cout=%d)",
                     gmax->K, (long long)M, Cout);
        p.gm.gmax = gmax->gmax; p.gm.gmin = gmax->gmin; p.gm.amax = gmax->amax; p.gm.amin = gmax->amin; p.gm.K = gmax->K; p.gm.sgn = gmax->sign_src;
        if (!y) {
            GemmArgs q = p;
            q.parts = gemm_parts(p.M);
            const int rc2 = a_mode == A_BNRELU ? stream_gemm_try(q, A_BNRELU, EPI_GMAX, vec, st) : 0;
            if (rc2 == 0) { set_error("papc_mlp_gemm_f32: y = NULL (no stored output under the max) is not built for a_mode=%d M=%lld Cin=%d Cout=%d K=%d", a_mode, (long long)M, Cin, Cout, gmax->K); return PAPC_E_UNSUPPORTED; }
            return rc2 < 0 ? rc2 : PAPC_OK;
        }
        switch (a_mode) {
        case A_PLAIN: return launch_gemm<A_PLAIN, EPI_STORE_GMAX>(p, vec, st);
        case A_BNRELU: return launch_gemm<A_BNRELU, EPI_STORE_GMAX>(p, vec, st);
        default: return launch_gemm<A_GROUP, EPI_STORE_GMAX>(p, vec, st);
        }
    }
    if (a_mode == A_XYZ) {
        GemmArgs q = p;
        q.parts = gemm_parts(p.M);
        const int rc2 = stream_gemm_try(q, A_XYZ, EPI_STORE, vec, st);
        if (rc2 == 0) { set_error("papc_mlp_gemm_f32: PAPC_A_XYZ is not built for M=%lld Cin=%d Cout=%d", (long long)M, Cin, Cout); return PAPC_E_UNSUPPORTED; }
        return rc2 < 0 ? rc2 : PAPC_OK;
    }
    switch (a_mode) {
    case A_PLAIN: return launch_gemm<A_PLAIN, EPI_STORE>(p, vec, st);
    case A_BNRELU: return launch_gemm<A_BNRELU, EPI_STORE>(p, vec, st);
    default: return launch_gemm<A_GROUP, EPI_STORE>(p, vec, st);
    }
}

int papc_mlp_gemm_rows_f32(int a_mode, const float *x, int64_t ldx, const papc_group_src *grp,
                           const float *bn_scale, const float *bn_shift, const float *w, const float *bias,
                           int64_t M, int Cin, int Cout, float *y, float *stats_partial, const papc_group_max *gmax,
                           const int32_t *rows_dev, papc_stream_t stream)
{
    return papc_mlp_gemm_rows_w_f32(a_mode, x, ldx, grp, bn_scale, bn_shift, w, bias, M, Cin, Cout, y, stats_partial, gmax, rows_dev, nullptr, stream);
}

int papc_mlp_xyz_ok(int64_t M, int C1, int C2)
{
    if (!knob(KNOB_STREAM) || knob(KNOB_GEMM_F32) || !knob(KNOB_DW_ROWS) || knob(KNOB_DW_F32)) return 0;
    if (M % 64 != 0 || M / 32 < knob(KNOB_STREAM_MINTILES)) return 0;
    if (C1 != 64 || !(C2 == 64 || C2 == 128)) return 0;
    if (M * (int64_t)C2 * 4 >= (1ll << 32)) return 0;
    if ((C1 / 64) * (C2 / 64) > knob(KNOB_DW_ROWS_BLOCKS)) return 0;
    return 1;
}

int papc_mlp_max_nostore_ok(int64_t M, int Cin, int Cout, int K)
{
    if (!knob(KNOB_STREAM) || knob(KNOB_GEMM_F32) || !knob(KNOB_STREAM_ASM) || !knob(KNOB_STREAM_MAXCAT) || !knob(KNOB_DW_ROWS) || knob(KNOB_DW_F32)) return 0;
    if (!knob(KNOB_MAX_NOSTORE)) return 0;
    if (M % 128 != 0 || M / 32 < knob(KNOB_STREAM_MINTILES) || M * (int64_t)Cout * 4 >= (1ll << 32)) return 0;
    if (!(K == 32 || K == 64 || K == 128) || !papc_mlp_gemm_gmax_ok(M, Cout, K)) return 0;
    if (!(Cin == 64 && Cout == 128)) return 0;
    return 1;
}

int papc_mlp_compact_ok(int64_t M, int K, int n_layers, const int *couts)
{
    if (!knob(KNOB_STREAM) || knob(KNOB_GEMM_F32) || !knob(KNOB_STREAM_ASM) || !knob(KNOB_DW_ROWSX) || knob(KNOB_DW_F32)) return 0;
    if (!couts || n_layers < 2 || M % 128 != 0 || M / 32 < knob(KNOB_STREAM_MINTILES) || K < 8 || K % 8 != 0) return 0;
    if (M * 256 * 4 >= (1ll << 32)) return 0;
    if (couts[0] != 128) return 0;
    for (int l = 1; l < n_layers; ++l)
        if (couts[l] != (l == n_layers - 1 ? 256 : 128)) return 0;
    return 1;
}

int papc_mlp_bwd_dx_f32(const papc_bwd_dy *dy, const float *wt, int64_t M, int Cin, int Cout, float *dx,
                        const papc_scatter_dst *scatter, const papc_bwd_red *next_red, papc_stream_t stream)
{
    PAPC_REQUIRE(wt, PAPC_E_INVALID, "papc_mlp_bwd_dx_f32: null wt");
    PAPC_REQUIRE(dx || scatter, PAPC_E_INVALID, "papc_mlp_bwd_dx_f32: need dx or scatter");
    PAPC_REQUIRE(M >= 1 && Cin >= 1 && Cout >= 1, PAPC_E_INVALID, "papc_mlp_bwd_dx_f32: bad sizes");
    PAPC_REQUIRE(M < (1ll << 31), PAPC_E_UNSUPPORTED, "papc_mlp_bwd_dx_f32: M=%lld >= 2^31 rows", (long long)M);
    bool vec = false;
    int rc = check_dy(dy, M, Cout, &vec, "papc_mlp_bwd_dx_f32");
    if (rc) return rc;
    GemmArgs p;
    memset(&p, 0, sizeof(p));
    fill_dy(p.a.d, dy);
    p.a.d.C = Cout;
    p.w = wt; p.ldw = Cout; p.M = M; p.Kin = Cout; p.Nout = Cin; p.y = dx; p.ldy = Cin;
    vec = vec && aligned16(wt);
    if (scatter) {
        PAPC_REQUIRE(scatter->grad_feats && scatter->D >= 1 && scatter->D + 3 == Cin, PAPC_E_INVALID,
                     "papc_mlp_bwd_dx_f32: scatter needs grad_feats and D+3 == Cin");
        PAPC_REQUIRE(scatter->N >= 1 && scatter->S >= 1 && scatter->K >= 1, PAPC_E_INVALID, "papc_mlp_bwd_dx_f32: scatter bad N/S/K");
        p.sc.gf = scatter->grad_feats; p.sc.idx = scatter->idx; p.sc.N = scatter->N; p.sc.S = scatter->S;
        p.sc.K = scatter->K; p.sc.D = scatter->D;
        p.sc.divSK = make_fastdiv((uint32_t)scatter->S * (uint32_t)scatter->K);
        p.sc.divK = make_fastdiv((uint32_t)scatter->K);
        p.nmap = scatter->col0 ? 1 : 0;
        p.a.g.D = scatter->D; p.a.g.xyz_first = scatter->col0 ? 1 : 0;
        p.Nout = scatter->D;
    }
    if (next_red) {
        PAPC_REQUIRE(!scatter && dx, PAPC_E_INVALID, "papc_mlp_bwd_dx_f32: next_red needs a dense dx");
        PAPC_REQUIRE(next_red->y && next_red->mean && next_red->invstd && next_red->scale && next_red->shift && next_red->red_partial,
                     PAPC_E_INVALID, "papc_mlp_bwd_dx_f32: null pointer in next_red");
        p.rd.y = next_red->y; p.rd.mean = next_red->mean; p.rd.invstd = next_red->invstd; p.rd.scale = next_red->scale;
        p.rd.shift = next_red->shift; p.stats = next_red->red_partial; p.rd.masked = next_red->store_masked ? 1 : 0;
    }
    const int tl_on = knob(KNOB_GEMM_TL);
    p.tl = tl_on && !scatter && dx && aligned16(dx) && Cin % 4 == 0 && (!next_red || (aligned16(next_red->y) && Cin <= 64 && !next_red->store_masked));
    hipStream_t st = as_stream(stream);
    ProfScope prof(PAPC_K_BWD_DX, st);
    if (next_red) {
        return dy->dz_mode == PAPC_DZ_DENSE ? launch_gemm<A_DY_DENSE, EPI_STORE_RED>(p, vec, st) : launch_gemm<A_DY_MAX, EPI_STORE_RED>(p, vec, st);
    }
// ... 72 lines not shown
```

### papc_amd/csrc/mlp_stream.hip

```cpp
#include "mlp_gemm.h"
#include <type_traits>
#include <utility>

namespace papc {

typedef float f32x4 __attribute__((ext_vector_type(4)));

template <int I, int N, class F>
__device__ __forceinline__ void sfor(F &&f)
{
    if constexpr (I < N) {
        f(std::integral_constant<int, I>{});
        sfor<I + 1, N>(f);
    }
}

template <bool ASM, int OFF, bool FIRST>
__device__ __forceinline__ void gload4(f32x4 &d, unsigned voff, const char *sbase)
{
    if constexpr (ASM) {
        if constexpr (FIRST) asm volatile("s_nop 4\n\tglobal_load_dwordx4 %0, %1, %2 offset:%3" : "+v"(d) : "v"(voff), "s"(sbase), "n"(OFF));
        else asm volatile("global_load_dwordx4 %0, %1, %2 offset:%3" : "+v"(d) : "v"(voff), "s"(sbase), "n"(OFF));
    } else {
        d = *reinterpret_cast<const f32x4 *>(sbase + voff + OFF);
    }
}
template <bool ASM, int N>
__device__ __forceinline__ void wait_vm()
{
    if constexpr (ASM) asm volatile("s_waitcnt vmcnt(%0)" ::"n"(N));
}
template <bool ASM>
__device__ __forceinline__ void touch(f32x4 &d)
{
    if constexpr (ASM) asm volatile("" : "+v"(d));
}

struct StreamGeo {
    int n_units;
    int ushift;
    int kgshift;
    const int *rows_dev;
    const float *wrow;
    const int *seg_grp;
    const float *wstat;
};

#ifndef PAPC_STREAM_PK
#define PAPC_STREAM_PK 1
#endif
__device__ __forceinline__ floatx2_t pk_fma(floatx2_t a, floatx2_t b, floatx2_t c) { return __builtin_elementwise_fma(a, b, c); }

template <int AMODE, int EPI, int KB16, int CK, int WN, bool ASM, bool CP = false, int KV = KB16 * 16, bool NR = false, int CBW = WN * 32, bool PS = false, int NWT = 8,
          bool GS = false>
__global__ __launch_bounds__(NWT * 64, NWT / 4) void stream_kernel(GemmArgs p, StreamGeo geo)
{
    static_assert(!GS || EPI == EPI_STORE_GMAX || EPI == EPI_GMAX, "GS: group-max epilogues only");
    static_assert(NWT == 8 || NWT == 12, "two or three waves per SIMD");
    static_assert(!PS || (CP && AMODE == A_DY_MAX), "PS: the compacted max-layer dX only (the one flavour where the result is bit-identical)");
    static_assert(!CP || ((AMODE == A_DY_DENSE || AMODE == A_DY_MAX) && EPI == EPI_STORE_RED && ASM && PAPC_STREAM_PK), "CP: dX flavours of the asm ring only");
    constexpr int NW = NWT;
    constexpr bool KR = (KV != KB16 * 16);
    constexpr int K = KR ? KV + 4 : KB16 * 16;
    constexpr int NT = WN * 32;
    constexpr int KBF = KR ? KB16 - 1 : KB16;
    static_assert(!KR || (KV == KB16 * 16 - 12 && !CP && PAPC_STREAM_PK && (AMODE == A_BNRELU || AMODE == A_DY_DENSE || AMODE == A_PLAIN)), "ragged k: four channels in the last block");
    static_assert(!NR || (EPI == EPI_STORE || EPI == EPI_STORE_RED), "ragged n: storing epilogues without the group max");
    constexpr int NCH = KBF / CK;
    static_assert(KBF % CK == 0 && NCH >= 2 && NCH % 2 == 0, "an even number of chunks per tile");
    constexpr bool DY = (AMODE == A_DY_DENSE || AMODE == A_DY_MAX);
    constexpr bool GM = (EPI == EPI_STORE_GMAX || EPI == EPI_GMAX);
    constexpr bool XYZ = (AMODE == A_XYZ);
    constexpr bool MC = (AMODE == A_MAXCAT);
    constexpr int KS = MC ? KB16 * 2 / 3 : 0;
    static_assert(!MC || (KB16 % 3 == 0 && CK == 1), "MAXCAT: Cout = 2 Cin, one k block per chunk");
    constexpr int NLD = (AMODE == A_DY_MAX) ? 6 : ((AMODE == A_DY_DENSE || MC) ? 4 : 2);
    constexpr int NLDP = KR ? NLD / 2 : 0;
    constexpr int CLB = CK * NLD;
    constexpr int CL = CLB + NLDP;
    static_assert(CL <= 60, "vmcnt is a 6-bit field");
    constexpr int ROWB = 6 * K + (KR ? 32 : 16);
    static_assert((ROWB / 16) % 2 == 1 && ROWB % 16 == 0, "conflict-free fragment reads");
    constexpr int NCST = (AMODE == A_BNRELU || MC) ? 2 : (DY ? 5 : (XYZ ? 4 : 0));
    constexpr bool CB = (CBW != NT);
    constexpr int TB = CBW / 32;
    static_assert(!CB || (NR && TB == WN - 1 && CBW % 32 != 0), "a narrow column block ends inside its last tile");
    constexpr int NROW = CB ? CBW + 1 : NT;
    constexpr int W_BYTES = NROW * ROWB;
    constexpr int CST_BYTES = NCST * K * 4 + (KR ? 32 : 0);
    constexpr bool XR = (EPI == EPI_XYZ_RED);
    constexpr int NSUM = XR ? 4 : 2;
    constexpr int RED_BYTES = NSUM * NW * NT * 4;
    constexpr int SMEM = (W_BYTES + CST_BYTES) > RED_BYTES ? (W_BYTES + CST_BYTES) : RED_BYTES;
    __shared__ __attribute__((aligned(16))) char smem[SMEM];
    char *cstb = smem + W_BYTES;

    const int tid = threadIdx.x, lane = tid & 63;
    const int wave = __builtin_amdgcn_readfirstlane(tid >> 6);
    const int hi = lane >> 5, l31 = lane & 31;
    const int n0 = blockIdx.y * CBW;
    const int ldx = (int)(DY ? p.a.d.C : p.a.ldx);
    auto nld_of = [](int ci) constexpr -> int { return MC ? ((ci % NCH) < KS ? 4 : 2) : (CK * NLD + ((ci % NCH) == NCH - 1 ? NLDP : 0)); };

    {
        const float *wb = p.w + (int64_t)n0 * p.ldw;
        constexpr int NP = NROW * (K / 4);
        constexpr int NI = (NP + NW * 64 - 1) / (NW * 64);
        constexpr bool PG = (NP % (NW * 64) != 0);
        static_assert(KR || CB || !PG || NW != 8, "whole float4 pieces per thread");
        float4 wv[NI];
#pragma unroll
        for (int q = 0; q < NI; ++q) {
            const int i = tid + q * NW * 64;
            const int n = i / (K / 4), k4 = (i - n * (K / 4)) * 4;
            bool ok = true;
            if constexpr (KR) ok = ok && k4 < KV;
            if constexpr (PG) ok = ok && i < NP;
            if constexpr (NR) ok = ok && n0 + n < p.Nout;
            if constexpr (CB) ok = ok && n < CBW;
            wv[q] = ok ? ld4(wb + (int64_t)n * p.ldw + k4) : make_float4(0.f, 0.f, 0.f, 0.f);
        }
#pragma unroll
        for (int q = 0; q < NI; ++q) {
            const int i = tid + q * NW * 64;
            const int n = i / (K / 4), k4 = (i - n * (K / 4)) * 4;
            uint2 q0, q1, q2;
            split3(wv[q], q0, q1, q2);
            char *d = smem + n * ROWB + k4 * 2;
            if (!PG || i < NP) {
                *reinterpret_cast<uint2 *>(d) = q0;
                *reinterpret_cast<uint2 *>(d + 2 * K) = q1;
                *reinterpret_cast<uint2 *>(d + 4 * K) = q2;
            }
        }
        if constexpr (KR) {
            for (int n = tid; n < NROW; n += NW * 64) {
                *reinterpret_cast<uint4 *>(smem + n * ROWB + 6 * K) = make_uint4(0u, 0u, 0u, 0u);
                *reinterpret_cast<uint4 *>(smem + n * ROWB + 6 * K + 16) = make_uint4(0u, 0u, 0u, 0u);
            }
        }
// ... 237 lines not shown
                }
                af[0] = __builtin_bit_cast(bf16x8, make_uint4(q0[0], q0[1], q0[2], q0[3]));
                af[1] = __builtin_bit_cast(bf16x8, make_uint4(q1[0], q1[1], q1[2], q1[3]));
                af[2] = __builtin_bit_cast(bf16x8, make_uint4(q2[0], q2[1], q2[2], q2[3]));
            }
#else
            float v[8];
            if constexpr (AMODE == A_PLAIN) {
#pragma unroll
                for (int i = 0; i < 4; ++i) { v[i] = r[0][i]; v[4 + i] = r[1][i]; }
            } else if constexpr (AMODE == A_BNRELU) {
                const f32x4 s0 = *reinterpret_cast<const f32x4 *>(cl + kb * 64), s1 = *reinterpret_cast<const f32x4 *>(cl + kb * 64 + 16);
                const f32x4 h0 = *reinterpret_cast<const f32x4 *>(cl + K * 4 + kb * 64), h1 = *reinterpret_cast<const f32x4 *>(cl + K * 4 + kb * 64 + 16);
#pragma unroll
                for (int i = 0; i < 4; ++i) {
                    v[i] = fmaxf(fmaf(s0[i], r[0][i], h0[i]), 0.f);
                    v[4 + i] = fmaxf(fmaf(s1[i], r[1][i], h1[i]), 0.f);
                }
            } else {
                f32x4 c[5][2];
#pragma unroll
                for (int q = 0; q < 5; ++q) {
                    c[q][0] = *reinterpret_cast<const f32x4 *>(cl + q * K * 4 + kb * 64);
                    c[q][1] = *reinterpret_cast<const f32x4 *>(cl + q * K * 4 + kb * 64 + 16);
                }
#pragma unroll
                for (int h = 0; h < 2; ++h)
#pragma unroll
                    for (int i = 0; i < 4; ++i) {
                        const float y = r[h][i];
                        float dz = r[2 + h][i];
                        if constexpr (AMODE == A_DY_MAX) dz = (__float_as_int(r[4 + h][i]) == kin) ? dz : 0.f;
                        const float z = fmaf(c[0][h][i], y, c[1][h][i]);
                        const float pp = z > 0.f ? dz : 0.f;
                        v[4 * h + i] = fmaf(-c[4][h][i], y - c[2][h][i], fmaf(c[0][h][i], pp, -c[3][h][i]));
                    }
            }
            split8(v, af);
#endif
            bf16x8 bq[WN][3];
#pragma unroll
            for (int wn = 0; wn < WN; ++wn)
#pragma unroll
                for (int pl = 0; pl < 3; ++pl)
                    bq[wn][pl] = *reinterpret_cast<const bf16x8 *>(((CB && wn == TB) ? wlb : wl + wn * 32 * ROWB) + pl * 2 * K + kb * 32);
#pragma unroll
            for (int t = 0; t < 6; ++t)
#pragma unroll
                for (int wn = 0; wn < WN; ++wn)
                    acc[wn] = __builtin_amdgcn_mfma_f32_32x32x16_bf16(af[BF16X3_PA[t]], bq[wn][BF16X3_PB[t]], acc[wn], 0, 0, 0);
        }
    };
    auto compute = [&](auto bi_, auto ci_) {
        constexpr int bi = decltype(bi_)::value, ci = decltype(ci_)::value;
        sfor<0, CK>([&](auto blk_) {
            constexpr int blk = decltype(blk_)::value;
            compute_block(std::integral_constant<int, ci * CK + blk>{}, &buf[bi][blk * NLD]);
        });
        if constexpr (KR && ci == NCH - 1) {
            const f32x4 z4 = f32x4{0.f, 0.f, 0.f, 0.f};
            f32x4 rr[4];
            rr[0] = pbuf[0]; rr[1] = z4;
            rr[2] = (AMODE == A_DY_DENSE) ? pbuf[NLDP - 1] : z4; rr[3] = z4;
            compute_block(std::integral_constant<int, KBF>{}, rr);
        }
    };

    float s1[WN], s2[WN], biasv[WN];
    float rsc[WN], rsh[WN], rmu[WN], ris[WN];
    float gmx[WN], gmn[WN];
    int gix[WN], gin[WN];
    float s3[WN], s4[WN];
    float4 kq[WN];
#pragma unroll
    for (int wn = 0; wn < WN; ++wn) {
        const int colr = n0 + wn * 32 + l31;
        const int col = NR ? min(colr, p.Nout - 1) : colr;
        s1[wn] = 0.f; s2[wn] = 0.f; s3[wn] = 0.f; s4[wn] = 0.f;
        kq[wn] = XR ? ld4(p.rd.scale + 4 * col) : make_float4(0.f, 0.f, 0.f, 0.f);
        biasv[wn] = (!CP && !(KR && DY) && p.bias && colr == col && (!CB || wn * 32 + l31 < CBW)) ? p.bias[col] : 0.f;
        rsc[wn] = rsh[wn] = rmu[wn] = ris[wn] = 0.f;
        if (EPI == EPI_STORE_RED) { rsc[wn] = p.rd.scale[col]; rsh[wn] = p.rd.shift[col]; rmu[wn] = p.rd.mean[col]; ris[wn] = p.rd.invstd[col]; }
        gmx[wn] = -INFINITY; gmn[wn] = INFINITY; gix[wn] = 0; gin[wn] = 0;
        if constexpr (GS) gin[wn] = (p.gm.sgn[col] < 0.f) ? (int)0x80000000u : 0;
    }

    auto epilogue = [&](int row0, int sub) {
        const int64_t ldy = p.ldy;
        if constexpr (XR) {
            const float4 *xq = reinterpret_cast<const float4 *>(p.rd.y) + row0 + 4 * hi;
#pragma unroll
            for (int g = 0; g < 4; ++g) {
                float4 xv[4];
#pragma unroll
                for (int i = 0; i < 4; ++i) xv[i] = xq[8 * g + i];
#pragma unroll
                for (int wn = 0; wn < WN; ++wn) {
#pragma unroll
                    for (int i = 0; i < 4; ++i) {
                        const int r = 4 * g + i;
                        const float z = fmaf(kq[wn].z, xv[i].z, fmaf(kq[wn].y, xv[i].y, fmaf(kq[wn].x, xv[i].x, kq[wn].w)));
                        const float pp = z > 0.f ? acc[wn][r] : 0.f;
                        s1[wn] = fmaf(pp, xv[i].x, s1[wn]); s2[wn] = fmaf(pp, xv[i].y, s2[wn]); s3[wn] = fmaf(pp, xv[i].z, s3[wn]);
                        s4[wn] += pp;
                        acc[wn][r] = 0.f;
                    }
                }
                __builtin_amdgcn_sched_barrier(0);
            }
            return;
        }
#pragma unroll
        for (int wn = 0; wn < WN; ++wn) {
            const int col = n0 + wn * 32 + l31;
            const bool cok = (!NR || col < p.Nout) && (!CB || wn * 32 + l31 < CBW);
            float *yp = p.y + (int64_t)(row0 + 4 * hi) * ldy + col;
            if (EPI == EPI_STORE_RED) {
                if (cok) {
                const float *qp = p.rd.y + (int64_t)(row0 + 4 * hi) * ldy + col;
                float yv[16];
#pragma unroll
                for (int r = 0; r < 16; ++r) yv[r] = qp[(int64_t)((r & 3) + 8 * (r >> 2)) * ldy];
#pragma unroll
                for (int r = 0; r < 16; ++r) {
                    const float v = acc[wn][r] + biasv[wn];
                    const float pp = fmaf(rsc[wn], yv[r], rsh[wn]) > 0.f ? v : 0.f;
                    if constexpr (CP) yp[(int64_t)((r & 3) + 8 * (r >> 2)) * ldy] = pp;
                    else yp[(int64_t)((r & 3) + 8 * (r >> 2)) * ldy] = v;
                    s1[wn] += pp;
                    s2[wn] = fmaf(pp, (yv[r] - rmu[wn]) * ris[wn], s2[wn]);
                    if constexpr (CP) { if ((r & 3) == 3) __builtin_amdgcn_sched_barrier(0); }
                }
                }
            } else {
#pragma unroll
                for (int r = 0; r < 16; ++r) {
                    const int ro = (r & 3) + 8 * (r >> 2);
                    const float v = acc[wn][r] + biasv[wn];
                    if (EPI != EPI_GMAX && cok) yp[(int64_t)ro * ldy] = v;
                    s1[wn] += v;
                    s2[wn] = fmaf(v, v, s2[wn]);
                    if (GM) {
                        const int off = sub * 32 + ro + 4 * hi;
                        if constexpr (GS) {
                            const float key = __int_as_float(__float_as_int(v) ^ gin[wn]);
                            if (key > gmx[wn]) { gmx[wn] = key; gix[wn] = off; }
                        } else {
                            if (v > gmx[wn]) { gmx[wn] = v; gix[wn] = off; }
                            if (v < gmn[wn]) { gmn[wn] = v; gin[wn] = off; }
                        }
                    }
                }
            }
#pragma unroll
            for (int r = 0; r < 16; ++r) acc[wn][r] = 0.f;
            if (GM && sub == U - 1) {
                if constexpr (GS) {
                    float vmx = gmx[wn];
                    int imx = gix[wn];
                    const float omx = __shfl_xor(vmx, 32);
                    const int oix = __shfl_xor(imx, 32);
                    if (omx > vmx || (omx == vmx && oix < imx)) { vmx = omx; imx = oix; }
                    if (hi == 0) {
                        const int64_t g = (int64_t)(row0 >> 5) >> geo.ushift;
                        const float sel = __int_as_float(__float_as_int(vmx) ^ gin[wn]);
                        p.gm.gmax[g * p.Nout + col] = sel; p.gm.amax[g * p.Nout + col] = imx;
                        p.gm.gmin[g * p.Nout + col] = sel; p.gm.amin[g * p.Nout + col] = imx;
                    }
                    gmx[wn] = -INFINITY; gix[wn] = 0;
                } else {
                float vmx = gmx[wn], vmn = gmn[wn];
                int imx = gix[wn], imn = gin[wn];
                const float omx = __shfl_xor(vmx, 32), omn = __shfl_xor(vmn, 32);
                const int oix = __shfl_xor(imx, 32), oin = __shfl_xor(imn, 32);
                if (omx > vmx || (omx == vmx && oix < imx)) { vmx = omx; imx = oix; }
                if (omn < vmn || (omn == vmn && oin < imn)) { vmn = omn; imn = oin; }
                if (hi == 0) {
                    const int64_t g = (int64_t)(row0 >> 5) >> geo.ushift;
                    p.gm.gmax[g * p.Nout + col] = vmx; p.gm.amax[g * p.Nout + col] = imx;
                    p.gm.gmin[g * p.Nout + col] = vmn; p.gm.amin[g * p.Nout + col] = imn;
                }
                gmx[wn] = -INFINITY; gmn[wn] = INFINITY; gix[wn] = 0; gin[wn] = 0;
                }
            }
        }
    };

    if constexpr (XYZ) {
        if (my_tiles > 0) {
            const float4 *xc = reinterpret_cast<const float4 *>(p.a.x);
            int row0 = tile_row0(0);
            float4 xn = xc[row0 + l31];
            for (int j = 0; j < my_tiles; ++j) {
                const float4 xv = xn;
                const int row0n = tile_row0(j + 1);
                xn = xc[row0n + l31];
                asm volatile("" ::: "memory");
                sfor<0, KB16>([&](auto kb_) { compute_xyz(kb_, xv); });
                epilogue(row0, j & (U - 1));
                row0 = row0n;
            }
        }
    }
    if (!XYZ && my_tiles > 0) {
        int row0 = tile_row0(0);
        SB sa = bases(row0);
        unsigned vgnxt = voff_grp0;
        auto vg_of = [&](int g) -> unsigned { return (unsigned)((g * ldx + 8 * hi) * 4); };
        if constexpr (CP) {
            const int r1 = tile_row0(1);
            wcur = -geo.wrow[row0 + l31];
            if constexpr (AMODE == A_DY_MAX) {
                sa.vg = vg_of(geo.seg_grp[(row0 + l31) >> 3]);
                vgnxt = vg_of(geo.seg_grp[(r1 + l31) >> 3]);
            }
        }
        issue(std::integral_constant<int, 0>{}, std::integral_constant<int, 0>{}, sa);
        issue(std::integral_constant<int, 1>{}, std::integral_constant<int, 1>{}, sa);
        wait_vm<ASM, nld_of(1)>();
        touch_buf(std::integral_constant<int, 0>{});
        for (int j = 0; j < my_tiles; ++j) {
            const int row0n = tile_row0(j + 1);
            SB sn = bases(row0n);
            if constexpr (CP) sn.vg = vgnxt;
// ... 27 lines not shown
            epilogue(row0, j & (U - 1));
            if constexpr (CP) {
                wcur = -wld;
                if constexpr (AMODE == A_DY_MAX) vgnxt = vg_of(gld);
            }
            if constexpr (LATE1) issue(std::integral_constant<int, 1>{}, std::integral_constant<int, 1>{}, sn);
            row0 = row0n;
            sa = sn;
        }
        wait_vm<ASM, 0>();
        touch_buf(std::integral_constant<int, 0>{});
        touch_buf(std::integral_constant<int, 1>{});
        touch_p();
    }

    if constexpr (EPI == EPI_STORE && (AMODE == A_BNRELU || AMODE == A_PLAIN) && !NR && !KR) {
        if (geo.wstat && p.stats && my_tiles > 0) {
            asm volatile("s_waitcnt vmcnt(0)" ::: "memory");
            for (int j = 0; j < my_tiles; ++j) {
                const int row0 = tile_row0(j);
                float cfq[2], vq[2][WN];
#pragma unroll
                for (int q = 0; q < 2; ++q) {
                    const int64_t row = row0 + 8 * (2 * q + hi);
                    cfq[q] = geo.wstat[row] - 1.f;
#pragma unroll
                    for (int wn = 0; wn < WN; ++wn) vq[q][wn] = p.y[row * p.ldy + n0 + wn * 32 + l31];
                }
#pragma unroll
                for (int q = 0; q < 2; ++q)
#pragma unroll
                    for (int wn = 0; wn < WN; ++wn) {
                        s1[wn] = fmaf(cfq[q], vq[q][wn], s1[wn]);
                        s2[wn] = fmaf(cfq[q] * vq[q][wn], vq[q][wn], s2[wn]);
                    }
            }
        }
    }

    if (p.stats) {
        __syncthreads();
        float *red = reinterpret_cast<float *>(smem);
#pragma unroll
        for (int wn = 0; wn < WN; ++wn) {
            s1[wn] += __shfl_xor(s1[wn], 32);
            s2[wn] += __shfl_xor(s2[wn], 32);
            if (XR) { s3[wn] += __shfl_xor(s3[wn], 32); s4[wn] += __shfl_xor(s4[wn], 32); }
            if (hi == 0) {
                red[(0 * NW + wave) * NT + wn * 32 + l31] = s1[wn];
                red[(1 * NW + wave) * NT + wn * 32 + l31] = s2[wn];
                if (XR) {
                    red[(2 * NW + wave) * NT + wn * 32 + l31] = s3[wn];
                    red[(3 * NW + wave) * NT + wn * 32 + l31] = s4[wn];
                }
            }
        }
        __syncthreads();
        for (int i = tid; i < NSUM * NT; i += NW * 64) {
            const int which = i / NT, c = i - which * NT;
            float t = 0.f;
#pragma unroll
            for (int w = 0; w < NW; ++w) t += red[(which * NW + w) * NT + c];
            const int64_t col_off = XR ? (int64_t)(n0 + c) * 4 + which : (int64_t)which * p.Nout + n0 + c;
            const int64_t row_ld = (int64_t)NSUM * p.Nout;
            if ((NR && n0 + c >= p.Nout) || (CB && c >= CBW)) continue;
            p.stats[(int64_t)blockIdx.x * row_ld + col_off] = t;
            for (int r = blockIdx.x + gridDim.x; r < p.parts; r += gridDim.x) p.stats[(int64_t)r * row_ld + col_off] = 0.f;
        }
    }
}

static int stream_ncu()
{
    static int ncu = 0;
    if (!ncu) {
        int dev = 0;
        hipDeviceProp_t prop;
        if (hipGetDevice(&dev) == hipSuccess && hipGetDeviceProperties(&prop, dev) == hipSuccess && prop.multiProcessorCount > 0) ncu = prop.multiProcessorCount;
        else ncu = 256;
    }
    return ncu;
}

template <int AMODE, int EPI, int KB16, int WN, bool CP = false, int KV = KB16 * 16, bool NR = false, int CBW = WN * 32, bool PS = false>
static int stream_go(const GemmArgs &p, const StreamGeo &geo, hipStream_t st)
{
    constexpr bool KR = (KV != KB16 * 16);
    constexpr int KBF = KR ? KB16 - 1 : KB16;
    constexpr int CK2 = (KBF == 6) ? 1 : 2;
    constexpr int CK = (KBF < 4 || AMODE == A_DY_MAX || AMODE == A_MAXCAT || (AMODE == A_DY_DENSE && (WN == 4 || KR)) || (AMODE == A_PLAIN && KB16 == 8 && WN == 4)) ? 1 : CK2;
    const int ncb = (p.Nout + CBW - 1) / CBW;
    int gx = std::max(8, (stream_ncu() / ncb) & ~7);
    if (!CP && (AMODE == A_MAXCAT || AMODE == A_XYZ)) gx *= 2;
    gx = std::min(gx, std::max(1, (geo.n_units + 7) / 8));
    if (gx > p.parts) gx = p.parts;
    dim3 grid((unsigned)gx, (unsigned)ncb);
    if constexpr (!CP && EPI == EPI_STORE_RED) { if (p.rd.masked) return 0; }
    if constexpr (CP) {
        if (!knob(KNOB_STREAM_ASM)) return 0;
        if constexpr (PS) {
            GemmArgs q = p;
            q.a.d.gout = p.a.d.psel;
            hipLaunchKernelGGL((stream_kernel<AMODE, EPI, KB16, CK, WN, true, true, KB16 * 16, false, WN * 32, true>), grid, dim3(512), 0, st, q, geo);
        } else {
            hipLaunchKernelGGL((stream_kernel<AMODE, EPI, KB16, CK, WN, true, true>), grid, dim3(512), 0, st, p, geo);
        }
        const int rc = check_launch("mlp stream gemm (compacted)");
        return rc ? rc : 1;
    }
    if constexpr (AMODE == A_XYZ) hipLaunchKernelGGL((stream_kernel<AMODE, EPI, KB16, CK, WN, false>), grid, dim3(512), 0, st, p, geo);
    else if (knob(KNOB_STREAM_ASM)) {
        if constexpr ((EPI == EPI_XYZ_RED || (EPI == EPI_STORE_RED && AMODE == A_DY_MAX && KB16 == 16)) && WN == 2 && !NR && KV == KB16 * 16) {
            if (knob(KNOB_STREAM_NW12)) hipLaunchKernelGGL((stream_kernel<AMODE, EPI, KB16, CK, WN, true, false, KV, NR, CBW, false, 12>), grid, dim3(768), 0, st, p, geo);
            else hipLaunchKernelGGL((stream_kernel<AMODE, EPI, KB16, CK, WN, true, false, KV, NR, CBW>), grid, dim3(512), 0, st, p, geo);
        } else if constexpr ((EPI == EPI_GMAX || EPI == EPI_STORE_GMAX) && !NR && KV == KB16 * 16) {
            if (p.gm.sgn) hipLaunchKernelGGL((stream_kernel<AMODE, EPI, KB16, CK, WN, true, false, KV, NR, CBW, false, 8, true>), grid, dim3(512), 0, st, p, geo);
            else hipLaunchKernelGGL((stream_kernel<AMODE, EPI, KB16, CK, WN, true, false, KV, NR, CBW>), grid, dim3(512), 0, st, p, geo);
        } else {
            hipLaunchKernelGGL((stream_kernel<AMODE, EPI, KB16, CK, WN, true, false, KV, NR, CBW>), grid, dim3(512), 0, st, p, geo);
        }
    }
    else if constexpr (AMODE == A_MAXCAT || EPI == EPI_GMAX || EPI == EPI_XYZ_RED || KR || NR) return 0;
    else hipLaunchKernelGGL((stream_kernel<AMODE, EPI, KB16, CK, WN, false>), grid, dim3(512), 0, st, p, geo);
    const int rc = check_launch("mlp stream gemm");
    return rc ? rc : 1;
}

template <int AMODE, int EPI>
static int stream_pick(const GemmArgs &p, const StreamGeo &geo, hipStream_t st)
{
    const int kb = p.Kin / 16;
    if (geo.wrow) {
        if constexpr (AMODE == A_DY_DENSE && EPI == EPI_STORE_RED) { if (kb == 8 && p.Nout == 128) return stream_go<AMODE, EPI, 8, 4, true>(p, geo, st); }
        if constexpr (AMODE == A_DY_MAX && EPI == EPI_STORE_RED) {
            if (kb == 16 && p.Nout == 128) {
                if (p.a.d.psel) return stream_go<AMODE, EPI, 16, 2, true, 256, false, 64, true>(p, geo, st);
                return stream_go<AMODE, EPI, 16, 2, true>(p, geo, st);
            }
        }
        return 0;
    }
    if (geo.wstat && (p.Kin == 196 || p.Nout == 196)) return 0;
    if (p.Kin == 196 || p.Nout == 196) {
        if constexpr (AMODE == A_BNRELU && EPI == EPI_STORE) { if (p.Kin == 128 && p.Nout == 196) return stream_go<AMODE, EPI, 8, 4, false, 128, true>(p, geo, st); }
        if constexpr (AMODE == A_BNRELU && (EPI == EPI_STORE_GMAX || EPI == EPI_STORE)) { if (p.Kin == 196 && p.Nout % 128 == 0) return stream_go<AMODE, EPI, 13, 4, false, 196>(p, geo, st); }
        if constexpr (AMODE == A_DY_MAX && EPI == EPI_STORE_RED) { if (p.Kin == 256 && p.Nout == 196) return stream_go<AMODE, EPI, 16, 4, false, 256, true, 98>(p, geo, st); }
        if constexpr (AMODE == A_DY_DENSE && EPI == EPI_STORE_RED) { if (p.Kin == 196 && p.Nout % 128 == 0) return stream_go<AMODE, EPI, 13, 4, false, 196>(p, geo, st); }
        return 0;
    }
    const int nt = p.Kin > 128 ? 64 : 128;
    int wn = std::min(p.Nout, nt) / 32;
    if (p.Nout % (32 * wn) != 0) {
        if (p.Nout == 96 && nt >= 96) wn = 3;
        else return 0;
    }
#define STREAM_CASE(KB, WNN) if (kb == KB && wn == WNN) return stream_go<AMODE, EPI, KB, WNN>(p, geo, st)
    if constexpr (EPI == EPI_GMAX) {
        STREAM_CASE(4, 4); STREAM_CASE(8, 4);
    } else if constexpr (AMODE == A_MAXCAT) {
        STREAM_CASE(12, 2); STREAM_CASE(24, 2);
    } else if constexpr (AMODE == A_XYZ) {
        STREAM_CASE(4, 2); STREAM_CASE(4, 4);
    } else if constexpr (AMODE == A_DY_DENSE && (EPI == EPI_STORE || EPI == EPI_XYZ_RED)) {
        STREAM_CASE(4, 2); STREAM_CASE(8, 2);
    } else {
        STREAM_CASE(2, 2); STREAM_CASE(2, 4);
        STREAM_CASE(4, 2); STREAM_CASE(4, 4);
        STREAM_CASE(8, 2); STREAM_CASE(8, 4);
        STREAM_CASE(4, 3); STREAM_CASE(8, 3);
        STREAM_CASE(6, 2); STREAM_CASE(6, 4);
        if constexpr (AMODE == A_DY_DENSE || AMODE == A_DY_MAX || AMODE == A_BNRELU) { STREAM_CASE(16, 2); }
    }
#undef STREAM_CASE
    return 0;
}

static int ilog2_exact(int v)
{
    int s = 0;
    while ((1 << s) < v) ++s;
    return (1 << s) == v ? s : -1;
}

int stream_gemm_try(const GemmArgs &p, int amode, int epi, bool vec, hipStream_t st)
{
    auto why = [&](int site) -> int { if (getenv("PAPC_STREAM_WHY")) fprintf(stderr, "[stream_gemm_try] declined at site %d: amode %d epi %d M %lld Kin %d Nout %d vec %d\n", site, amode, epi, (long long)p.M, p.Kin, p.Nout, (int)vec); return 0; };
    if (!knob(KNOB_STREAM) || knob(KNOB_GEMM_F32) || !vec) return why(1);
    if (p.M % 32 != 0 || p.M / 32 < knob(KNOB_STREAM_MINTILES)) return why(2);
    if (((p.Kin % 32 != 0 || p.Nout % 32 != 0) && p.Kin != 196 && p.Nout != 196) || p.Kin % 4 != 0 || p.Kin < 32 || p.Kin > (amode == A_MAXCAT ? 384 : 256) || p.Nout < 64) return why(3);
    if (amode == A_MAXCAT && (p.a.d.C != 2 * p.Nout || p.Kin != 3 * p.Nout || p.a.ldx != p.Nout)) return why(4);
    if (p.wmap || p.nmap || p.ldy != p.Nout) return why(5);
    if (!(p.stats || epi == EPI_STORE)) return why(6);
    StreamGeo geo;
    geo.ushift = 0; geo.kgshift = 5;
    geo.rows_dev = p.rows_dev; geo.wrow = nullptr; geo.seg_grp = nullptr;
    geo.wstat = (p.rows_dev && epi == EPI_STORE && (amode == A_BNRELU || amode == A_PLAIN)) ? p.wstat : nullptr;
    if (p.wstat && !geo.wstat) return why(12);
    if (amode == A_DY_DENSE || amode == A_DY_MAX) { geo.wrow = p.a.d.wrow; geo.seg_grp = p.a.d.seg_grp; geo.rows_dev = p.a.d.rows_dev; }
    if (geo.rows_dev && (p.M % 128 != 0 || epi == EPI_STORE_GMAX || epi == EPI_GMAX)) return why(7);
    if (geo.wrow && (!geo.rows_dev || (amode == A_DY_MAX && !geo.seg_grp))) return why(8);
    if (epi == EPI_STORE_GMAX || epi == EPI_GMAX) {
        const int s = ilog2_exact(p.gm.K);
        if (s < 5 || p.M % p.gm.K != 0) return why(9);
        geo.ushift = s - 5;
    }
    if ((amode == A_DY_MAX && !geo.wrow) || amode == A_MAXCAT) {
        const int s = ilog2_exact(p.a.d.K);
        if (s < 5) return why(10);
        geo.kgshift = s;
    }
    geo.n_units = (int)((p.M / 32) >> geo.ushift);
    if (amode == A_BNRELU && epi == EPI_STORE) return stream_pick<A_BNRELU, EPI_STORE>(p, geo, st);
    if (amode == A_BNRELU && epi == EPI_GMAX) return knob(KNOB_STREAM_ASM) ? stream_pick<A_BNRELU, EPI_GMAX>(p, geo, st) : 0;
    if (amode == A_BNRELU && epi == EPI_STORE_GMAX) return stream_pick<A_BNRELU, EPI_STORE_GMAX>(p, geo, st);
    if (amode == A_PLAIN && epi == EPI_STORE) return stream_pick<A_PLAIN, EPI_STORE>(p, geo, st);
    if (amode == A_DY_DENSE && epi == EPI_STORE_RED) return stream_pick<A_DY_DENSE, EPI_STORE_RED>(p, geo, st);
    if (amode == A_DY_DENSE && epi == EPI_STORE) return stream_pick<A_DY_DENSE, EPI_STORE>(p, geo, st);
    if (amode == A_DY_DENSE && epi == EPI_XYZ_RED) return (knob(KNOB_STREAM_ASM) && !geo.rows_dev) ? stream_pick<A_DY_DENSE, EPI_XYZ_RED>(p, geo, st) : 0;
    if (amode == A_XYZ && epi == EPI_STORE) return stream_pick<A_XYZ, EPI_STORE>(p, geo, st);
    if (amode == A_MAXCAT && epi == EPI_STORE_RED) return stream_pick<A_MAXCAT, EPI_STORE_RED>(p, geo, st);
    if (amode == A_DY_MAX && epi == EPI_STORE_RED) return stream_pick<A_DY_MAX, EPI_STORE_RED>(p, geo, st);
    return why(11);
}

}
```

### papc_amd/csrc/sa_mlp.hip

```cpp
#include "common.h"

#define SA_CALL(expr)                 \
    do {                              \
        const int rc__ = (expr);      \
        if (rc__ != PAPC_OK) return rc__; \
    } while (0)

namespace papc {
int pfn_gram_stats(const float *features, const int32_t *num_voxels, const int32_t *coors, int P, int T, float vx, float vy, float x_offset, float y_offset, int zero_padded,
                   double *gram_partial, const float *w, int C, const float *gamma, const float *beta, float eps, float momentum, float *mean, float *invstd,
                   float *scale, float *shift, float *running_mean, float *running_var, double *gram, unsigned *ticket, hipStream_t st);
int pfn_gram_impl(const float *features, const int32_t *num_voxels, const int32_t *coors, int P, int T, float vx, float vy, float x_offset, float y_offset,
                  double *gram_partial, int zero_padded, papc_stream_t stream);
int pfn_apply_impl(const float *features, const int32_t *num_voxels, const int32_t *coors, int P, int T, float vx, float vy, float x_offset, float y_offset,
                   const float *w, int C, const float *scale, const float *shift, float *out, int32_t *argmax, int zero_padded, papc_stream_t stream);
int pfn_bwd_sparse_impl(const float *features, const int32_t *num_voxels, const int32_t *coors, int P, int T, float vx, float vy, float x_offset, float y_offset,
                        const float *w, int C, const float *gout, const int32_t *argmax, const float *mean, const float *invstd, const float *scale,
                        const float *shift, float *partial, int zero_padded, papc_stream_t stream);
int pfn_bwd_fold_finalize(const float *partial, int n_chunks, float *sums, int64_t M, const float *w, int C, const double *gram, const float *mean,
                          const float *invstd, const float *scale, float *dgamma, float *dbeta, float *dw, int flags, unsigned *ticket, hipStream_t st);

constexpr int A_PLAIN_ = PAPC_A_PLAIN, A_BNRELU_ = PAPC_A_BNRELU, A_GROUP_ = PAPC_A_GROUP, A_XYZ_ = PAPC_A_XYZ;

struct Carver {
    char *base;
    size_t off;
    template <class T>
    T *take(size_t n)
    {
        off = (off + 255) & ~(size_t)255;
        T *p = base ? reinterpret_cast<T *>(base + off) : nullptr;
        off += n * sizeof(T);
        return p;
    }
};

struct SavedPtrs {
    float *y[PAPC_SA_MAX_LAYERS];
    float *cst[PAPC_SA_MAX_LAYERS];
    int32_t *argmax;
    float *gbuf_f;
    float *xc; double *gram; float *wf;
    float *P;
};
struct FwdPtrs {
    float *stats;
    int32_t *gbuf_i;
    float *P, *wfeat;
    double *gpart;
};
struct BwdPtrs {
    float *c12[PAPC_SA_MAX_LAYERS];
    float *wt[PAPC_SA_MAX_LAYERS];
    float *part[PAPC_SA_MAX_LAYERS];
    float *red, *fused_red[2];
    float *dz[2];
    float *psel, *wcat, *hb, *eq, *dwmax_ws;
    float *bpart;
    float *dwx_part, *Gs, *part_g, *wft;
    float *tmp_gb;
};

static inline int64_t rows_of(const papc_sa_desc &d) { return (int64_t)d.B * d.S * d.K; }

static bool defer_fold(const papc_sa_grads &gr, const float *partial, int n_chunks, int64_t ld, int rows, int cols, float *out, int64_t out_ld, int accumulate)
{
    papc_fold_list *fl = gr.defer;
    if (!fl || !fl->jobs || fl->count >= fl->capacity) return false;
    papc_fold_job &j = fl->jobs[fl->count++];
    j.partial = partial; j.n_chunks = n_chunks; j.accumulate = accumulate; j.ld = ld; j.rows = rows; j.cols = cols; j.out = out; j.out_ld = out_ld;
    return true;
}
static bool defer_room(const papc_sa_grads &gr, int n) { return gr.defer && gr.defer->jobs && gr.defer->count + n <= gr.defer->capacity; }
static inline int cin_of(const papc_sa_plan &p, int l) { return l == 0 ? p.cin0 : p.d.cout[l - 1]; }

static int dw_rows_per_chunk(int64_t M, int cout, int cin, int min_rows = 256)
{
    const bool wide = cin > 128 && cin <= 160;
    const int tiles = ((cout + 127) / 128) * (wide ? 1 : (cin + 127) / 128);
    const int want = std::max(1, 512 / tiles);
    int64_t rpc = (M + want - 1) / want;
    rpc = std::max<int64_t>(min_rows, ((rpc + 63) / 64) * 64);
    return (int)rpc;
}

static int dw_chunk(const papc_sa_plan &p, int l, int a_mode, int dz_mode)
{
    const int64_t M = rows_of(p.d);
    int rpc = 0;
    const bool plain = p.d.input == PAPC_SA_IN_ROWS;
    if (l > 0 || !plain) rpc = papc_mlp_bwd_dw_chunk_hint(M, cin_of(p, l), p.d.cout[l], a_mode, dz_mode, dz_mode == PAPC_DZ_MAX ? p.d.K : 0);
    if (rpc <= 0) rpc = dw_rows_per_chunk(M, p.d.cout[l], cin_of(p, l));
    return rpc;
}

static size_t layout_saved(const papc_sa_plan &p, void *base, SavedPtrs &s)
{
    Carver c{reinterpret_cast<char *>(base), 0};
    const int L = p.d.n_layers;
    const int64_t M = rows_of(p.d), G = (int64_t)p.d.B * p.d.S;
    memset(&s, 0, sizeof(s));
    for (int l = 0; l < L; ++l) {
        const bool stored = !(l == 0 && p.xyz1) && !(l == L - 1 && p.nostore);
        s.y[l] = stored ? c.take<float>((size_t)M * p.d.cout[l] + 64) : nullptr;
        s.cst[l] = c.take<float>(4 * (size_t)p.d.cout[l]);
    }
    if (p.d.pool) {
        s.argmax = c.take<int32_t>((size_t)G * p.d.cout[L - 1]);
        if (p.gmax || p.compact) s.gbuf_f = c.take<float>(2 * (size_t)G * p.d.cout[L - 1]);
    }
    if (p.xyz1) {
        s.xc = c.take<float>((size_t)M * 4);
        s.gram = c.take<double>(16);
        s.wf = c.take<float>(4 * (size_t)p.d.cout[0]);
    }
    if (p.lin0) s.P = c.take<float>((size_t)p.d.B * p.d.N * p.d.cout[0]);
    return c.off;
}

static size_t layout_fwd(const papc_sa_plan &p, void *base, FwdPtrs &f)
{
    Carver c{reinterpret_cast<char *>(base), 0};
    const int L = p.d.n_layers;
    const int64_t M = rows_of(p.d), G = (int64_t)p.d.B * p.d.S;
    memset(&f, 0, sizeof(f));
    int cmax = 0;
    for (int l = 0; l < L; ++l) cmax = std::max(cmax, p.d.cout[l]);
    const int rows = std::max(papc_mlp_gemm_parts(M), p.lin0 ? papc_lingather_parts(M) : 0) + (p.compact ? papc_compact_corr_parts() : 0);
    f.stats = c.take<float>((size_t)rows * 2 * cmax * L);
    if (p.gmax) f.gbuf_i = c.take<int32_t>(2 * (size_t)G * p.d.cout[L - 1]);
    if (p.lin0) f.wfeat = c.take<float>((size_t)p.d.cout[0] * p.d.D);
    if (p.xyz1) f.gpart = c.take<double>((size_t)papc_xyz_parts(M) * 16 + 16);
    return c.off;
}

static size_t layout_bwd(const papc_sa_plan &p, void *base, BwdPtrs &b)
{
    Carver c{reinterpret_cast<char *>(base), 0};
    const int L = p.d.n_layers;
    const int64_t M = rows_of(p.d), G = (int64_t)p.d.B * p.d.S;
    memset(&b, 0, sizeof(b));
    int cmax = p.cin0;
    for (int l = 0; l < L; ++l) cmax = std::max(cmax, p.d.cout[l]);
    const int n_parts = (int)std::min<int64_t>(512, (M + 127) / 128);
    const int gparts = papc_mlp_gemm_parts(M);
    for (int l = 0; l < L; ++l) {
        const int cin = cin_of(p, l), cout = p.d.cout[l];
        b.c12[l] = c.take<float>(2 * (size_t)cout);
        b.wt[l] = c.take<float>((size_t)cin * cout);
        const int dzm = (l == L - 1 && p.d.pool) ? PAPC_DZ_MAX : PAPC_DZ_DENSE;
        const int am = l == 0 ? (p.d.input == PAPC_SA_IN_ROWS ? A_PLAIN_ : A_GROUP_) : ((l == 1 && p.xyz1) ? A_XYZ_ : A_BNRELU_);
        const int rpc = dw_chunk(p, l, am, dzm);
        const int64_t n_chunks = (M + rpc - 1) / rpc;
        b.part[l] = c.take<float>((size_t)n_chunks * ((size_t)cout * cin + cout));
    }
    b.red = c.take<float>((size_t)n_parts * 2 * cmax);
    b.fused_red[0] = c.take<float>((size_t)gparts * 2 * cmax);
    b.fused_red[1] = c.take<float>((size_t)gparts * 2 * cmax);
    if (L > 1 || p.d.input == PAPC_SA_IN_ROWS) {
        b.dz[0] = c.take<float>((size_t)M * cmax + 64);
        if (L > 2) b.dz[1] = c.take<float>((size_t)M * cmax + 64);
    }
    if (p.d.pool && L > 1) {
        const int cL = p.d.cout[L - 1], cLi = p.d.cout[L - 2];
        b.psel = c.take<float>((size_t)G * cL);
        b.wcat = c.take<float>((size_t)cLi * (cL + cLi));
        b.hb = c.take<float>((size_t)cLi);
        b.eq = c.take<float>(2 * (size_t)cL);
        if (p.nostore) b.dwmax_ws = c.take<float>((size_t)papc_mlp_bwd_dw_max_ws_floats(M, cLi, cL) + 4);
    }
    if (p.xyz1) b.bpart = c.take<float>((size_t)std::max(papc_xyz_bwd_parts(M), papc_mlp_gemm_parts(M)) * p.d.cout[0] * 4);
    if (p.lin0) {
        const int c0 = p.d.cout[0];
        const int64_t BN = (int64_t)p.d.B * p.d.N;
        b.dwx_part = c.take<float>((size_t)std::max(papc_lingather_parts(M), papc_lingather_list_parts(BN)) * c0 * 3);
        b.Gs = c.take<float>((size_t)BN * c0);
        const int rpc_g = dw_rows_per_chunk(BN, c0, p.d.D, 64);
        b.part_g = c.take<float>((size_t)((BN + rpc_g - 1) / rpc_g) * ((size_t)c0 * p.d.D + c0));
        b.wft = c.take<float>((size_t)p.d.D * c0);
    }
    b.tmp_gb = c.take<float>(2 * (size_t)cmax);
    return c.off;
}

constexpr int PG_GROUP = 128, PG_MAX_ROWS = 16384;
struct PlanesSaved {
    float *y[PAPC_SA_MAX_LAYERS], *cst[PAPC_SA_MAX_LAYERS];
    int32_t *argmax; float *gbuf_f;
    float *ysel;
    void *PT[PAPC_SA_MAX_LAYERS];
    void *wtp[PAPC_SA_MAX_LAYERS];
};
struct PlanesFwd { void *wp[PAPC_SA_MAX_LAYERS]; void *P; float *stats[PAPC_SA_MAX_LAYERS]; int32_t *gbuf_i; };
struct PlanesBwd { void *dyp, *dypt; float *dz[2], *red[3], *part[PAPC_SA_MAX_LAYERS], *tmp_gb; };

static int pg_split_for(int R1, int R2, int nst)
{
    const int tiles = ((R1 + 127) / 128) * ((R2 + 127) / 128);
    int s = 1;
    const int min_stages = tiles <= 2 ? 2 : 8;
    while (s * 2 * tiles <= 256 && nst % (s * 2) == 0 && nst / (s * 2) >= min_stages) s *= 2;
    return s;
}
static inline int pg_n_in(const papc_sa_plan &p) { return p.d.input == PAPC_SA_IN_ROWS ? p.cin0 : p.d.D; }

static size_t layout_planes_saved(const papc_sa_plan &p, void *base, PlanesSaved &s)
{
    Carver c{reinterpret_cast<char *>(base), 0};
    const int L = p.d.n_layers;
    const int64_t M = rows_of(p.d), T = M / PG_GROUP;
    memset(&s, 0, sizeof(s));
    for (int l = 0; l < L; ++l) {
        s.y[l] = c.take<float>((size_t)M * p.d.cout[l]);
        s.cst[l] = c.take<float>(4 * (size_t)p.d.cout[l]);
    }
// ... 218 lines not shown
    PAPC_REQUIRE(M < (1ll << 31), PAPC_E_UNSUPPORTED, "papc_sa_mlp_plan: >= 2^31 rows");
    for (int l = 0; l < d.n_layers; ++l) PAPC_REQUIRE(d.cout[l] >= 1, PAPC_E_INVALID, "papc_sa_mlp_plan: cout[%d] = %d", l, d.cout[l]);
    memset(plan, 0, sizeof(*plan));
    plan->d = d;
    const int L = d.n_layers;
    const bool plain = d.input == PAPC_SA_IN_ROWS, ev = d.eval_bn != 0;
    plan->cin0 = plain ? d.cin : d.D + 3;
    PAPC_REQUIRE(plan->cin0 >= 1, PAPC_E_INVALID, "papc_sa_mlp_plan: no input channels");
    const bool has_idx = !plain && d.identity_rows == 0, has_feats = !plain && d.D > 0;
    {
        bool ok = !(d.disable & PAPC_SA_NO_PLANES) && !ev && !has_idx && M % PG_GROUP == 0 && M >= PG_GROUP && M <= PG_MAX_ROWS && L >= 2;
        ok = ok && (d.pool ? (d.K % PG_GROUP == 0 && d.K / PG_GROUP <= 64) : (plain && !(d.disable & PAPC_SA_NO_PLANES_POINTWISE)));
        for (int l = 0; l < L; ++l) ok = ok && d.cout[l] % 8 == 0;
        ok = ok && (plain ? plan->cin0 % 8 == 0 : d.S == 1);
        plan->planes = ok ? 1 : 0;
    }
    if (plan->planes) {
        PlanesSaved ps; PlanesFwd pf; PlanesBwd pb;
        char *fake = reinterpret_cast<char *>((uintptr_t)1 << 40);
        layout_planes_saved(*plan, fake, ps);
        for (int l = 0; l < PAPC_SA_MAX_LAYERS; ++l) {
            plan->off_y[l] = l < L ? (int64_t)(reinterpret_cast<char *>(ps.y[l]) - fake) : -1;
            plan->off_cst[l] = l < L ? (int64_t)(reinterpret_cast<char *>(ps.cst[l]) - fake) : -1;
        }
        plan->off_argmax = ps.argmax ? (int64_t)(reinterpret_cast<char *>(ps.argmax) - fake) : -1;
        plan->saved_bytes = (int64_t)layout_planes_saved(*plan, nullptr, ps) + 256;
        plan->fwd_scratch_bytes = (int64_t)layout_planes_fwd(*plan, nullptr, pf) + 256;
        plan->bwd_scratch_bytes = (int64_t)layout_planes_bwd(*plan, nullptr, pb) + 256;
        return PAPC_OK;
    }
    plan->lin0 = !(d.disable & PAPC_SA_NO_LINGATHER) && !ev && !plain && has_idx && has_feats && L >= 2 && d.D % 4 == 0 && d.D >= 16 &&
                 d.cout[0] % 4 == 0 && d.cout[0] <= 256;
    plan->xyz1 = !(d.disable & PAPC_SA_NO_XYZ1) && !ev && !plain && has_idx && !has_feats && d.D == 0 && L >= 3 &&
                 papc_mlp_xyz_ok(M, d.cout[0], d.cout[1]);
    plan->compact = plan->lin0 && d.pool && !(d.disable & PAPC_SA_NO_COMPACT) && io && io->compact && papc_mlp_compact_ok(M, d.K, L, d.cout);
    const int cL = d.cout[L - 1], cLi = L > 1 ? d.cout[L - 2] : plan->cin0;
    plan->gmax = !plan->compact && d.pool && !(d.disable & PAPC_SA_NO_GMAX) && !ev && papc_mlp_gemm_gmax_ok(M, cL, d.K);
    plan->nostore = plan->gmax && !(d.disable & PAPC_SA_NO_NOSTORE) && L >= 2 && !(L == 2 && plan->xyz1) && papc_mlp_max_nostore_ok(M, cLi, cL, d.K);
    plan->sparse_max = plan->nostore;
    SavedPtrs s; FwdPtrs f; BwdPtrs b;
    {
        char *fake = reinterpret_cast<char *>((uintptr_t)1 << 40);
        layout_saved(*plan, fake, s);
        for (int l = 0; l < PAPC_SA_MAX_LAYERS; ++l) {
            plan->off_y[l] = (l < L && s.y[l]) ? (int64_t)(reinterpret_cast<char *>(s.y[l]) - fake) : -1;
            plan->off_cst[l] = (l < L && s.cst[l]) ? (int64_t)(reinterpret_cast<char *>(s.cst[l]) - fake) : -1;
        }
        plan->off_argmax = s.argmax ? (int64_t)(reinterpret_cast<char *>(s.argmax) - fake) : -1;
    }
    plan->saved_bytes = (int64_t)layout_saved(*plan, nullptr, s) + 256;
    plan->fwd_scratch_bytes = (int64_t)layout_fwd(*plan, nullptr, f) + 256;
    plan->bwd_scratch_bytes = (int64_t)layout_bwd(*plan, nullptr, b) + 256;
    return PAPC_OK;
}

int papc_sa_mlp_fwd(const papc_sa_plan *plan, const papc_sa_io *io, papc_stream_t st)
{
    PAPC_REQUIRE(plan && io && io->out && io->saved && io->scratch, PAPC_E_INVALID, "papc_sa_mlp_fwd: null pointer");
    const papc_sa_plan &p = *plan;
    const papc_sa_desc &d = p.d;
    const int L = d.n_layers;
    const int64_t M = rows_of(d), G = (int64_t)d.B * d.S;
    const bool plain = d.input == PAPC_SA_IN_ROWS, ev = d.eval_bn != 0;
    PAPC_REQUIRE(plain ? io->x_rows != nullptr : (io->xyz && io->new_xyz), PAPC_E_INVALID, "papc_sa_mlp_fwd: missing input");
    PAPC_REQUIRE(plain || d.identity_rows || io->idx, PAPC_E_INVALID, "papc_sa_mlp_fwd: grouped input without idx (set identity_rows for sample_and_group_all)");
    PAPC_REQUIRE(plain || d.D == 0 || io->feats, PAPC_E_INVALID, "papc_sa_mlp_fwd: D = %d but feats is NULL", d.D);
    PAPC_REQUIRE(!p.compact || io->compact, PAPC_E_INVALID, "papc_sa_mlp_fwd: the plan is compacted but io->compact is NULL");
    if (p.planes) {
        for (int l = 0; l < L; ++l) PAPC_REQUIRE(io->layer[l].w && io->layer[l].gamma && io->layer[l].beta, PAPC_E_INVALID, "papc_sa_mlp_fwd: layer %d lacks w / gamma / beta", l);
        return planes_fwd(p, *io, st);
    }
    SavedPtrs s; FwdPtrs f;
    layout_saved(p, io->saved, s);
    layout_fwd(p, io->scratch, f);
    const int parts = papc_mlp_gemm_parts(M);
    const bool wstats = p.compact && !(d.disable & PAPC_SA_NO_WSTATS);
    const int R_c = (p.compact && !wstats) ? papc_compact_corr_parts() : 0;
    papc_group_src grp;
    if (!plain) fill_grp(grp, d, *io, p.compact);
    if (!plain && wstats) grp.wstat = io->compact->wrow;
    int cmax = 0;
    for (int l = 0; l < L; ++l) cmax = std::max(cmax, d.cout[l]);
    const size_t stats_stride = (size_t)(std::max(parts, p.lin0 ? papc_lingather_parts(M) : 0) + R_c) * 2 * cmax;

    const float *prev_y = nullptr, *prev_sc = nullptr, *prev_sh = nullptr;
    int cin = p.cin0;
    const float *xc = nullptr;
    papc_group_max gm;
    memset(&gm, 0, sizeof(gm));
    for (int l = 0; l < L; ++l) {
        const papc_sa_layer &ly = io->layer[l];
        PAPC_REQUIRE(ly.w && ly.gamma && ly.beta, PAPC_E_INVALID, "papc_sa_mlp_fwd: layer %d lacks w / gamma / beta", l);
        PAPC_REQUIRE(!ev || (ly.running_mean && ly.running_var), PAPC_E_INVALID, "papc_sa_mlp_fwd: eval_bn needs the running statistics");
        const int cout = d.cout[l];
        float *stats = ev ? nullptr : f.stats + (size_t)l * stats_stride;
        int parts_l = parts;
        const papc_group_max *gm_ref = nullptr;
        if (l == L - 1 && p.gmax) {
            gm.gmax = s.gbuf_f; gm.gmin = s.gbuf_f + G * cout; gm.amax = f.gbuf_i; gm.amin = f.gbuf_i + G * cout; gm.K = d.K;
            gm.sign_src = (d.disable & PAPC_SA_NO_GSIGN) ? nullptr : ly.gamma;
            gm_ref = &gm;
        }
        float *y = s.y[l];
        float *cst = s.cst[l];
        if (l == 0 && p.xyz1) {
            const double *gpart1;
            if (io->xc && io->xc_gram) { xc = io->xc; gpart1 = io->xc_gram; }
            else {
                SA_CALL(papc_xyz_group_f32(&grp, d.B, s.xc, f.gpart + 16, st));
                SA_CALL(papc_xyz_gram_fold_f32(f.gpart + 16, papc_xyz_parts(M), f.gpart, st));
                xc = s.xc; gpart1 = f.gpart;
            }
            SA_CALL(papc_xyz_l1_finalize_f32(gpart1, 1, M, ly.w, cin, 0, ly.b, ly.gamma, ly.beta, d.eps, d.momentum, cout, cst, cst + cout, cst + 2 * cout,
                                             cst + 3 * cout, ly.running_mean, ly.running_var, s.wf, s.gram, st));
            prev_y = nullptr; prev_sc = cst + 2 * cout; prev_sh = cst + 3 * cout;
            cin = cout;
            continue;
        }
        if (l == 1 && p.xyz1) {
            SA_CALL(papc_mlp_gemm_f32(A_XYZ_, xc, 4, nullptr, s.wf, nullptr, ly.w, ly.b, M, cin, cout, y, stats, gm_ref, st));
        } else if (l == 0 && plain) {
            SA_CALL(papc_mlp_gemm_f32(A_PLAIN_, io->x_rows, cin, nullptr, nullptr, nullptr, ly.w, ly.b, M, cin, cout, y, stats, gm_ref, st));
        } else if (l == 0 && p.lin0) {
            const int fcol0 = d.xyz_first ? 3 : 0;
            const float *wfeat = io->wfeat;
            if (!wfeat) {
                SA_CALL(papc_copy2d_f32(ly.w + fcol0, cin, f.wfeat, d.D, cout, d.D, 0, st));
                wfeat = f.wfeat;
            }
            const int64_t BN = (int64_t)d.B * d.N;
            SA_CALL(papc_mlp_gemm_f32(A_PLAIN_, io->feats, d.D, nullptr, nullptr, nullptr, wfeat, nullptr, BN, d.D, cout, s.P, nullptr, nullptr, st));
            parts_l = papc_lingather_parts(M);
            SA_CALL(papc_lingather_fwd_f32(s.P, &grp, d.B, ly.w, cin, d.xyz_first ? 0 : d.D, ly.b, cout, y, stats, st));
        } else if (l == 0) {
            SA_CALL(papc_mlp_gemm_f32(A_GROUP_, nullptr, 0, &grp, nullptr, nullptr, ly.w, ly.b, M, cin, cout, y, stats, gm_ref, st));
        } else if (p.compact) {
            SA_CALL(papc_mlp_gemm_rows_w_f32(A_BNRELU_, prev_y, cin, nullptr, prev_sc, prev_sh, ly.w, ly.b, M, cin, cout, y, stats, nullptr, io->compact->rows,
                                             wstats ? io->compact->wrow : nullptr, st));
        } else {
            SA_CALL(papc_mlp_gemm_f32(A_BNRELU_, prev_y, cin, nullptr, prev_sc, prev_sh, ly.w, ly.b, M, cin, cout, y, stats, gm_ref, st));
        }
        if (p.compact && !wstats) {
            SA_CALL(papc_bn_stats_corr_f32(y, cout, io->compact->start, io->compact->coef, io->compact->G, stats + (size_t)parts_l * 2 * cout, st));
            parts_l += R_c;
        }
        if (ev) SA_CALL(papc_bn_eval_consts_f32(ly.running_mean, ly.running_var, ly.gamma, ly.beta, d.eps, cout, cst, cst + cout, cst + 2 * cout, cst + 3 * cout, st));
        else SA_CALL(papc_bn_finalize_f32(stats, parts_l, M, cout, ly.gamma, ly.beta, d.eps, d.momentum, cst, cst + cout, cst + 2 * cout, cst + 3 * cout,
                                          ly.running_mean, ly.running_var, st));
        prev_y = y; prev_sc = cst + 2 * cout; prev_sh = cst + 3 * cout;
        cin = cout;
    }
    if (!d.pool) return papc_bn_relu_f32(prev_y, prev_sc, prev_sh, M, cin, io->out, st);
    if (p.compact) return papc_bn_relu_max_seg_f32(prev_y, cin, io->compact->start, prev_sc, prev_sh, (int)G, io->out, s.argmax, s.gbuf_f, st);
    if (p.gmax) return papc_bn_select_max_f32(s.gbuf_f, s.gbuf_f + G * cin, f.gbuf_i, f.gbuf_i + G * cin, prev_sc, prev_sh, G, cin, io->out, s.argmax, st);
    return papc_bn_relu_max_f32(prev_y, prev_sc, prev_sh, G, d.K, cin, io->out, s.argmax, st);
}

int papc_sa_mlp_bwd(const papc_sa_plan *plan, const papc_sa_io *io, const papc_sa_grads *gr, papc_stream_t st)
{
    PAPC_REQUIRE(plan && io && gr && gr->gout && io->saved && io->scratch, PAPC_E_INVALID, "papc_sa_mlp_bwd: null pointer");
    const papc_sa_plan &p = *plan;
    const papc_sa_desc &d = p.d;
    const int L = d.n_layers;
    const int64_t M = rows_of(d), G = (int64_t)d.B * d.S;
    const bool plain = d.input == PAPC_SA_IN_ROWS, ev = d.eval_bn != 0;
    if (p.planes) return planes_bwd(p, *io, *gr, st);
    SavedPtrs s; BwdPtrs b;
    layout_saved(p, io->saved, s);
    layout_bwd(p, io->scratch, b);
    const float *xc = p.xyz1 ? ((io->xc && io->xc_gram) ? io->xc : s.xc) : nullptr;
    papc_group_src grp;
    if (!plain) fill_grp(grp, d, *io, p.compact);
    const int n_parts = (int)std::min<int64_t>(512, (M + 127) / 128);
    const int gemm_parts = papc_mlp_gemm_parts(M);
    const bool x_needs = plain && gr->grad_x, f_needs = !plain && d.D > 0 && gr->grad_feats && !d.cut_gather_grad;
    const float *ysel = (p.gmax || p.compact) ? s.gbuf_f : nullptr;
    const float *ones = io->consts3, *zeros = nullptr, *big = nullptr;
    int cmaxc = 0;
    for (int l = 0; l < L; ++l) cmaxc = std::max(cmaxc, d.cout[l]);
    if (p.lin0) {
        PAPC_REQUIRE(io->consts3 && io->consts3_ld >= d.cout[0], PAPC_E_INVALID, "papc_sa_mlp_bwd: the gather-add first layer needs consts3 (ones | zeros | 1e30 rows of >= %d floats)", d.cout[0]);
        zeros = io->consts3 + io->consts3_ld; big = io->consts3 + 2 * (int64_t)io->consts3_ld;
    }

    bool need_wt[PAPC_SA_MAX_LAYERS];
    const float *wts[PAPC_SA_MAX_LAYERS];
    for (int l = 0; l < L; ++l) {
        need_wt[l] = l > 0 || x_needs || f_needs;
        wts[l] = nullptr;
    }
    if (p.sparse_max) need_wt[L - 1] = false;
    if (p.lin0) need_wt[0] = false;
    {
        const float *srcs[8]; float *dsts[8]; int rws[8], cls[8];
        int n = 0;
        for (int l = 0; l < L; ++l) {
            if (!need_wt[l]) continue;
            if (gr->wt[l]) { wts[l] = gr->wt[l]; continue; }
            srcs[n] = io->layer[l].w; dsts[n] = b.wt[l]; rws[n] = d.cout[l]; cls[n] = cin_of(p, l);
            wts[l] = b.wt[l];
            if (++n == 8) { SA_CALL(papc_transpose_batch_f32(srcs, dsts, rws, cls, n, st)); n = 0; }
        }
        if (n) SA_CALL(papc_transpose_batch_f32(srcs, dsts, rws, cls, n, st));
    }

    papc_reduce_job jobs[PAPC_SA_MAX_LAYERS];
    int n_jobs = 0;
    bool xyz_fused = false;
    bool dz0_masked = false;
    const float *dz = nullptr;
    const float *fused_red = nullptr;
    int flip = 0;
    for (int l = L - 1; l >= 0; --l) {
        const papc_sa_layer &ly = io->layer[l];
        const int cout = d.cout[l], cin = cin_of(p, l);
        const float *cst = s.cst[l];
        float *c12 = b.c12[l];
        const bool acc_w = gr->acc_w[l] != 0, acc_gb = gr->acc_gb[l] != 0 && !ev;
        float *dgamma = gr->dgamma[l] ? gr->dgamma[l] : b.tmp_gb, *dbeta = gr->dbeta[l] ? gr->dbeta[l] : b.tmp_gb + cmaxc;
        PAPC_REQUIRE(gr->dw[l], PAPC_E_INVALID, "papc_sa_mlp_bwd: dw[%d] is NULL", l);
        papc_bwd_dy dy;
        memset(&dy, 0, sizeof(dy));
        if (p.compact) { dy.wrow = io->compact->wrow; dy.seg_grp = io->compact->seg_grp; dy.rows_dev = io->compact->rows; }
        if (l == L - 1 && !d.pool) { dy.dz_mode = PAPC_DZ_DENSE; dy.dz = gr->gout; dy.K = 1; }
        else if (l == L - 1) { dy.dz_mode = PAPC_DZ_MAX; dy.gout = gr->gout; dy.argmax = s.argmax; dy.K = d.K; }
        else { dy.dz_mode = PAPC_DZ_DENSE; dy.dz = dz; dy.K = 1; }
        if (l == 0 && p.xyz1) {
            PAPC_REQUIRE(!gr->dgamma[l] || (gr->acc_gb[l] != 0) == (gr->acc_w[l] != 0), PAPC_E_UNSUPPORTED,
                         "papc_sa_mlp_bwd: the coordinates-only first layer takes ONE accumulate flag for dw / dgamma / dbeta");
            int nbp = papc_xyz_bwd_parts(M);
            if (xyz_fused) nbp = papc_mlp_gemm_parts(M);
            else SA_CALL(papc_xyz_l1_bwd_f32(dz, xc, s.wf, M, cout, b.bpart, st));
            SA_CALL(papc_xyz_l1_bwd_finalize_f32(b.bpart, nbp, M, cout, s.gram, ly.w, cin, 0, ly.b, cst, cst + cout, cst + 2 * cout, dgamma, dbeta, gr->dw[l],
                                                 acc_w ? 1 : 0, st));
            if (gr->db[l] && !acc_w) SA_CALL(papc_fill_f32(gr->db[l], cout, 0.f, st));
// ... 204 lines not shown
```

Before: 21850.

## Fuse per-segment max into compacted last-layer GEMM epilogue via atomic keys

For the compacted SA path, the last MLP layer's GEMM epilogue now computes per-segment, per-channel max (sign-adjusted by gamma) and merges it into a 64-bit value|row key buffer with atomic max. A new select kernel then reads these keys to produce the BN+ReLU pooled output and argmax, scanning rows only when the BN scale sign disagrees with gamma. The key buffer is zeroed inside a combined BN-finalize kernel for the preceding layer, which avoids a separate memset launch. The aim is to skip re-reading the large last-layer activation for max pooling, at the cost of global atomics and extra epilogue work.

```diff
diff --git a/include/papc_hip.h b/include/papc_hip.h
--- a/include/papc_hip.h
+++ b/include/papc_hip.h
@@ -443,6 +443,12 @@
 int papc_bn_stats_corr_f32(const float *y, int C, const int32_t *start, const float *coef, int G, float *stats_rows, papc_stream_t stream);
 int papc_bn_relu_max_seg_f32(const float *y, int C, const int32_t *start, const float *scale, const float *shift, int G, float *out,
                              int32_t *argmax, float *ysel, papc_stream_t stream);
+int papc_mlp_seg_epi_ok(int64_t M, int Cin, int Cout);
+int papc_mlp_gemm_rows_keys_f32(const float *x, int64_t ldx, const float *bn_scale, const float *bn_shift, const float *w, const float *bias,
+                                int64_t M, int Cin, int Cout, float *y, float *stats_partial, const int32_t *rows_dev, const float *wrow,
+                                const int32_t *seg_grp, const float *sign_src, unsigned long long *keys, papc_stream_t stream);
+int papc_bn_relu_select_seg_f32(const unsigned long long *keys, const float *y, int C, const int32_t *start, const float *sign_src,
+                                const float *scale, const float *shift, int G, float *out, int32_t *argmax, float *ysel, papc_stream_t stream);
 int papc_lingather_fwd_f32(const float *P, const papc_group_src *grp, int B, const float *w, int ldw, int xcol0, const float *bias, int C,
                            float *y, float *stats_partial, papc_stream_t stream);
 int papc_lingather_bwd_f32(const papc_bwd_dy *dy, const papc_group_src *grp, int B, int C, float *G, float *dwx_partial, papc_stream_t stream);
diff --git a/papc_amd/_lib.py b/papc_amd/_lib.py
--- a/papc_amd/_lib.py
+++ b/papc_amd/_lib.py
@@ -92,6 +92,9 @@
     "papc_mlp_compact_ok": (c_i, [c_l, c_i, c_i, c_p]),
     "papc_bn_stats_corr_f32": (c_i, [c_p, c_i, c_p, c_p, c_i, c_p, c_p]),
     "papc_bn_relu_max_seg_f32": (c_i, [c_p, c_i, c_p, c_p, c_p, c_i, c_p, c_p, c_p, c_p]),
+    "papc_mlp_seg_epi_ok": (c_i, [c_l, c_i, c_i]),
+    "papc_mlp_gemm_rows_keys_f32": (c_i, [c_p, c_l, c_p, c_p, c_p, c_p, c_l, c_i, c_i, c_p, c_p, c_p, c_p, c_p, c_p, c_p, c_p]),
+    "papc_bn_relu_select_seg_f32": (c_i, [c_p, c_p, c_i, c_p, c_p, c_p, c_p, c_i, c_p, c_p, c_p, c_p]),
     "papc_bn_select_max_f32": (c_i, [c_p, c_p, c_p, c_p, c_p, c_p, c_l, c_i, c_p, c_p, c_p]),
     "papc_bn_finalize_f32": (c_i, [c_p, c_i, c_l, c_i, c_p, c_p, c_f, c_f, c_p, c_p, c_p, c_p, c_p, c_p, c_p]),
     "papc_bn_relu_max_f32": (c_i, [c_p, c_p, c_p, c_l, c_i, c_i, c_p, c_p, c_p]),
diff --git a/papc_amd/csrc/bn_ops.hip b/papc_amd/csrc/bn_ops.hip
--- a/papc_amd/csrc/bn_ops.hip
+++ b/papc_amd/csrc/bn_ops.hip
@@ -57,12 +57,12 @@
     s1 = t1; s2 = t2;
 }
 
-__global__ __launch_bounds__(64) void bn_finalize_kernel(const float *__restrict__ part, int n_tiles, int64_t M, int C,
-                                                        const float *__restrict__ gamma, const float *__restrict__ beta,
-                                                        float eps, float momentum, float *mean, float *invstd, float *scale,
-                                                        float *shift, float *rmean, float *rvar)
-{
-    const int c = blockIdx.x, tl = threadIdx.x;
+__device__ __forceinline__ void bn_finalize_channel(const int c, const float *__restrict__ part, int n_tiles, int64_t M, int C,
+                                                    const float *__restrict__ gamma, const float *__restrict__ beta,
+                                                    float eps, float momentum, float *mean, float *invstd, float *scale,
+                                                    float *shift, float *rmean, float *rvar)
+{
+    const int tl = threadIdx.x;
     const float gam = gamma ? gamma[c] : 1.f, bet = beta ? beta[c] : 0.f;
     const float rm0 = rmean ? rmean[c] : 0.f, rv0 = rvar ? rvar[c] : 0.f;
     double s1 = 0.0, s2 = 0.0;
@@ -81,6 +81,30 @@
         if (rmean) rmean[c] = momentum * rm0 + (1.f - momentum) * (float)mu;
         if (rvar) rvar[c] = momentum * rv0 + (1.f - momentum) * (float)var;
     }
+}
+__global__ __launch_bounds__(64) void bn_finalize_kernel(const float *__restrict__ part, int n_tiles, int64_t M, int C,
+                                                        const float *__restrict__ gamma, const float *__restrict__ beta,
+                                                        float eps, float momentum, float *mean, float *invstd, float *scale,
+                                                        float *shift, float *rmean, float *rvar)
+{
+    bn_finalize_channel(blockIdx.x, part, n_tiles, M, C, gamma, beta, eps, momentum, mean, invstd, scale, shift, rmean, rvar);
+}
+constexpr int BN_CLEAR_PER_LANE = 16, BN_CLEAR_PER_WG = 64 * BN_CLEAR_PER_LANE;
+__global__ __launch_bounds__(64) void bn_finalize_clear_kernel(const float *__restrict__ part, int n_tiles, int64_t M, int C,
+                                                              const float *__restrict__ gamma, const float *__restrict__ beta,
+                                                              float eps, float momentum, float *mean, float *invstd, float *scale,
+                                                              float *shift, float *rmean, float *rvar, uint4 *__restrict__ clr, int64_t n16)
+{
+    if ((int)blockIdx.x >= C) {
+        const int64_t i0 = (int64_t)((int)blockIdx.x - C) * BN_CLEAR_PER_WG + threadIdx.x;
+#pragma unroll
+        for (int q = 0; q < BN_CLEAR_PER_LANE; ++q) {
+            const int64_t i = i0 + q * 64;
+            if (i < n16) clr[i] = make_uint4(0u, 0u, 0u, 0u);
+        }
+        return;
+    }
+    bn_finalize_channel(blockIdx.x, part, n_tiles, M, C, gamma, beta, eps, momentum, mean, invstd, scale, shift, rmean, rvar);
 }
 
 template <int V>
@@ -543,6 +567,20 @@
     }
 }
 
+int bn_finalize_clear(const float *stats_partial, int n_tiles, int64_t M, int C, const float *gamma, const float *beta, float eps, float momentum,
+                      float *mean, float *invstd, float *scale, float *shift, float *running_mean, float *running_var, void *clr, int64_t bytes,
+                      hipStream_t st)
+{
+    PAPC_REQUIRE(stats_partial && mean && invstd && scale && shift && clr, PAPC_E_INVALID, "bn_finalize_clear: null pointer");
+    PAPC_REQUIRE(n_tiles >= 1 && M >= 1 && C >= 1 && bytes >= 16 && bytes % 16 == 0 && aligned16(clr), PAPC_E_INVALID, "bn_finalize_clear: bad sizes");
+    const int64_t n16 = bytes / 16, nclr = cdiv(n16, BN_CLEAR_PER_WG);
+    PAPC_REQUIRE(nclr + C < (1ll << 31), PAPC_E_UNSUPPORTED, "bn_finalize_clear: %lld bytes", (long long)bytes);
+    ProfScope prof(PAPC_K_MISC, st);
+    hipLaunchKernelGGL(bn_finalize_clear_kernel, dim3((unsigned)(C + nclr)), dim3(64), 0, st, stats_partial, n_tiles, M, C, gamma, beta, eps, momentum,
+                       mean, invstd, scale, shift, running_mean, running_var, reinterpret_cast<uint4 *>(clr), n16);
+    return check_launch("bn_finalize_clear");
+}
+
 }
 
 
diff --git a/papc_amd/csrc/capi.hip b/papc_amd/csrc/capi.hip
--- a/papc_amd/csrc/capi.hip
+++ b/papc_amd/csrc/capi.hip
@@ -70,6 +70,7 @@
     {"PAPC_LG_PP", 1, 0, 1},
     {"PAPC_PG_GROUP", 1, 0, 1},
     {"PAPC_PG_PIPE", 1, 0, 1},
+    {"PAPC_SEG_EPI", 1, 0, 1},
 };
 static int g_knobs[KNOB_COUNT];
 static int knob_parse(int id, const char *e)
diff --git a/papc_amd/csrc/common.h b/papc_amd/csrc/common.h
--- a/papc_amd/csrc/common.h
+++ b/papc_amd/csrc/common.h
@@ -24,7 +24,7 @@
 enum Knob {
     KNOB_LG_PARTS, KNOB_DW_F32, KNOB_DW_DBG, KNOB_DW_XYZ, KNOB_PARTS, KNOB_GEMM_F32, KNOB_GEMM_WAVES, KNOB_MAXCAT_WAVES,
     KNOB_GEMM_WS, KNOB_GEMM_OCC, KNOB_GEMM_DBG, KNOB_GEMM_KB, KNOB_GEMM_MINWG, KNOB_GEMM_TL, KNOB_FPS_THREADS,
-    KNOB_FPS_THREADS_SMALL, KNOB_STREAM, KNOB_STREAM_MINTILES, KNOB_STREAM_CK, KNOB_STREAM_ASM, KNOB_PFN_MFMA, KNOB_DW_RS64, KNOB_DW_ROWS, KNOB_DW_ROWS_BLOCKS, KNOB_DW_ROWSX, KNOB_PG_DBG, KNOB_PG_NB, KNOB_PG_NS, KNOB_STREAM_MAXCAT, KNOB_MAX_NOSTORE, KNOB_PFN_FUSED_TAILS, KNOB_STREAM_NW12, KNOB_LG_LISTS, KNOB_FOLD_WAVES, KNOB_LGL_VARIANT, KNOB_LG_PP, KNOB_PG_GROUP, KNOB_PG_PIPE, KNOB_COUNT
+    KNOB_FPS_THREADS_SMALL, KNOB_STREAM, KNOB_STREAM_MINTILES, KNOB_STREAM_CK, KNOB_STREAM_ASM, KNOB_PFN_MFMA, KNOB_DW_RS64, KNOB_DW_ROWS, KNOB_DW_ROWS_BLOCKS, KNOB_DW_ROWSX, KNOB_PG_DBG, KNOB_PG_NB, KNOB_PG_NS, KNOB_STREAM_MAXCAT, KNOB_MAX_NOSTORE, KNOB_PFN_FUSED_TAILS, KNOB_STREAM_NW12, KNOB_LG_LISTS, KNOB_FOLD_WAVES, KNOB_LGL_VARIANT, KNOB_LG_PP, KNOB_PG_GROUP, KNOB_PG_PIPE, KNOB_SEG_EPI, KNOB_COUNT
 };
 int knob(int id);
 
diff --git a/papc_amd/csrc/compact.hip b/papc_amd/csrc/compact.hip
--- a/papc_amd/csrc/compact.hip
+++ b/papc_amd/csrc/compact.hip
@@ -166,6 +166,56 @@
     *reinterpret_cast<float4 *>(ysel + q) = make_float4(ys[0], ys[1], ys[2], ys[3]);
 }
 
+__global__ __launch_bounds__(256) void seg_select_kernel(const unsigned long long *__restrict__ keys, const float *__restrict__ y, int C,
+                                                         const int32_t *__restrict__ start, const float *__restrict__ sign_src,
+                                                         const float *__restrict__ scale, const float *__restrict__ shift, int G,
+                                                         float *__restrict__ out, int32_t *__restrict__ argmax, float *__restrict__ ysel)
+{
+    const int CQ = C >> 2;
+    const int64_t e = (int64_t)blockIdx.x * 256 + threadIdx.x;
+    if (e >= (int64_t)G * CQ) return;
+    const int g = (int)(e / CQ), c = (int)(e - (int64_t)g * CQ) * 4;
+    const int r0 = start[g], r1 = start[g + 1];
+    const int64_t q = (int64_t)g * C + c;
+    const float4 sc = *reinterpret_cast<const float4 *>(scale + c), sh = *reinterpret_cast<const float4 *>(shift + c);
+    const float4 gm = *reinterpret_cast<const float4 *>(sign_src + c);
+    const ulonglong2 k01 = *reinterpret_cast<const ulonglong2 *>(keys + q), k23 = *reinterpret_cast<const ulonglong2 *>(keys + q + 2);
+    const float s4[4] = {sc.x, sc.y, sc.z, sc.w}, h4[4] = {sh.x, sh.y, sh.z, sh.w}, g4[4] = {gm.x, gm.y, gm.z, gm.w};
+    const unsigned long long k4[4] = {k01.x, k01.y, k23.x, k23.y};
+    int flip[4], am[4];
+    bool scan[4];
+    float ys[4], o[4];
+#pragma unroll
+    for (int i = 0; i < 4; ++i) {
+        flip[i] = s4[i] >= 0.f ? 0 : (int)0x80000000u;
+        scan[i] = flip[i] != (g4[i] < 0.f ? (int)0x80000000u : 0);
+        const int row = (int)~(unsigned)k4[i];
+        const unsigned u = (unsigned)(k4[i] >> 32);
+        const bool hit = !scan[i] && u > 0x007FFFFFu && row >= r0 && row < r1;
+        am[i] = hit ? row : r0;
+        const int kb = (u & 0x80000000u) ? (int)(u ^ 0x80000000u) : (int)~u;
+        ys[i] = hit ? __int_as_float(kb ^ flip[i]) : __int_as_float((int)0xFF800000u ^ flip[i]);
+        if (hit && kb == 0) ys[i] = y[(int64_t)row * C + c + i];
+    }
+#pragma unroll
+    for (int i = 0; i < 4; ++i) {
+        if (scan[i]) {
+            float mx = -INFINITY;
+            int ix = r0;
+            for (int r = r0; r < r1; ++r) {
+                const float k = __int_as_float(__float_as_int(y[(int64_t)r * C + c + i]) ^ flip[i]);
+                if (k > mx) { mx = k; ix = r; }
+            }
+            ys[i] = __int_as_float(__float_as_int(mx) ^ flip[i]);
+            am[i] = ix;
+        }
+        o[i] = relu_np(fmaf(s4[i], ys[i], h4[i]));
+    }
+    *reinterpret_cast<float4 *>(out + q) = make_float4(o[0], o[1], o[2], o[3]);
+    *reinterpret_cast<int4 *>(argmax + q) = make_int4(am[0], am[1], am[2], am[3]);
+    *reinterpret_cast<float4 *>(ysel + q) = make_float4(ys[0], ys[1], ys[2], ys[3]);
+}
+
 }
 
 using namespace papc;
@@ -212,4 +262,18 @@
     return check_launch("papc_bn_relu_max_seg_f32");
 }
 
-}
+int papc_bn_relu_select_seg_f32(const unsigned long long *keys, const float *y, int C, const int32_t *start, const float *sign_src, const float *scale,
+                                const float *shift, int G, float *out, int32_t *argmax, float *ysel, papc_stream_t stream)
+{
+    PAPC_REQUIRE(keys && y && start && sign_src && scale && shift && out && argmax && ysel, PAPC_E_INVALID, "papc_bn_relu_select_seg_f32: null pointer");
+    PAPC_REQUIRE(G >= 1 && C >= 4 && C % 4 == 0, PAPC_E_UNSUPPORTED, "papc_bn_relu_select_seg_f32: C=%d must be a multiple of 4", C);
+    PAPC_REQUIRE(aligned16(keys) && aligned16(sign_src) && aligned16(scale) && aligned16(shift) && aligned16(out) && aligned16(argmax) && aligned16(ysel),
+                 PAPC_E_INVALID, "papc_bn_relu_select_seg_f32: 16-byte alignment");
+    hipStream_t st = as_stream(stream);
+    ProfScope prof(PAPC_K_BN_RELU_MAX, st);
+    hipLaunchKernelGGL(seg_select_kernel, dim3((unsigned)cdiv((int64_t)G * (C / 4), 256)), dim3(256), 0, st, keys, y, C, start, sign_src, scale, shift, G,
+                       out, argmax, ysel);
+    return check_launch("papc_bn_relu_select_seg_f32");
+}
+
+}
diff --git a/papc_amd/csrc/mlp_gemm.h b/papc_amd/csrc/mlp_gemm.h
--- a/papc_amd/csrc/mlp_gemm.h
+++ b/papc_amd/csrc/mlp_gemm.h
@@ -18,6 +18,8 @@
 struct GmaxDst {
     float *gmax, *gmin; int32_t *amax, *amin; int K;
     const float *sgn;
+    unsigned long long *keys;
+    const int32_t *seg;
 };
 
 struct GemmArgs {
diff --git a/papc_amd/csrc/mlp_gemm.hip b/papc_amd/csrc/mlp_gemm.hip
--- a/papc_amd/csrc/mlp_gemm.hip
+++ b/papc_amd/csrc/mlp_gemm.hip
@@ -911,10 +911,11 @@
     return papc_mlp_gemm_rows_f32(a_mode, x, ldx, grp, bn_scale, bn_shift, w, bias, M, Cin, Cout, y, stats_partial, gmax, nullptr, stream);
 }
 
-int papc_mlp_gemm_rows_w_f32(int a_mode, const float *x, int64_t ldx, const papc_group_src *grp,
-                           const float *bn_scale, const float *bn_shift, const float *w, const float *bias,
-                           int64_t M, int Cin, int Cout, float *y, float *stats_partial, const papc_group_max *gmax,
-                           const int32_t *rows_dev, const float *wrow, papc_stream_t stream)
+static int gemm_rows_impl(int a_mode, const float *x, int64_t ldx, const papc_group_src *grp,
+                          const float *bn_scale, const float *bn_shift, const float *w, const float *bias,
+                          int64_t M, int Cin, int Cout, float *y, float *stats_partial, const papc_group_max *gmax,
+                          const int32_t *rows_dev, const float *wrow, const int32_t *seg_grp, const float *sign_src,
+                          unsigned long long *keys, papc_stream_t stream)
 {
     PAPC_REQUIRE(w && (y || gmax), PAPC_E_INVALID, "papc_mlp_gemm_f32: null w/y");
     PAPC_REQUIRE(!rows_dev || (!gmax && (a_mode == A_PLAIN || a_mode == A_BNRELU)), PAPC_E_UNSUPPORTED,
@@ -928,6 +929,8 @@
     p.w = w; p.ldw = Cin; p.bias = bias; p.M = M; p.Kin = Cin; p.Nout = Cout; p.y = y; p.ldy = Cout; p.stats = stats_partial;
     p.rows_dev = rows_dev;
     p.wstat = rows_dev ? wrow : nullptr;
+    p.gm.keys = keys; p.gm.seg = seg_grp;
+    if (keys) p.gm.sgn = sign_src;
     p.wmap = (a_mode == A_GROUP) ? 1 : 0;
     const bool vec = p.a.vec && (p.wmap || (aligned16(w) && Cin % 4 == 0));
     hipStream_t st = as_stream(stream);
@@ -964,6 +967,32 @@
     case A_BNRELU: return launch_gemm<A_BNRELU, EPI_STORE>(p, vec, st);
     default: return launch_gemm<A_GROUP, EPI_STORE>(p, vec, st);
     }
+}
+
+int papc_mlp_gemm_rows_w_f32(int a_mode, const float *x, int64_t ldx, const papc_group_src *grp,
+                           const float *bn_scale, const float *bn_shift, const float *w, const float *bias,
+                           int64_t M, int Cin, int Cout, float *y, float *stats_partial, const papc_group_max *gmax,
+                           const int32_t *rows_dev, const float *wrow, papc_stream_t stream)
+{
+    return gemm_rows_impl(a_mode, x, ldx, grp, bn_scale, bn_shift, w, bias, M, Cin, Cout, y, stats_partial, gmax, rows_dev, wrow, nullptr, nullptr, nullptr, stream);
+}
+
+int papc_mlp_seg_epi_ok(int64_t M, int Cin, int Cout)
+{
+    if (!knob(KNOB_STREAM) || knob(KNOB_GEMM_F32) || !knob(KNOB_STREAM_ASM)) return 0;
+    if (M % 128 != 0 || M / 32 < knob(KNOB_STREAM_MINTILES)) return 0;
+    return Cin == 128 && Cout >= 128 && Cout % 128 == 0;
+}
+
+int papc_mlp_gemm_rows_keys_f32(const float *x, int64_t ldx, const float *bn_scale, const float *bn_shift, const float *w, const float *bias,
+                                int64_t M, int Cin, int Cout, float *y, float *stats_partial, const int32_t *rows_dev, const float *wrow,
+                                const int32_t *seg_grp, const float *sign_src, unsigned long long *keys, papc_stream_t stream)
+{
+    PAPC_REQUIRE(y && rows_dev && seg_grp && sign_src && keys, PAPC_E_INVALID, "papc_mlp_gemm_rows_keys_f32: null pointer");
+    PAPC_REQUIRE(((uintptr_t)keys & 7) == 0 && ((uintptr_t)seg_grp & 3) == 0, PAPC_E_INVALID, "papc_mlp_gemm_rows_keys_f32: keys must be 8-byte aligned");
+    PAPC_REQUIRE(papc_mlp_seg_epi_ok(M, Cin, Cout), PAPC_E_UNSUPPORTED, "papc_mlp_gemm_rows_keys_f32: not built for M=%lld Cin=%d Cout=%d (papc_mlp_seg_epi_ok)",
+                 (long long)M, Cin, Cout);
+    return gemm_rows_impl(PAPC_A_BNRELU, x, ldx, nullptr, bn_scale, bn_shift, w, bias, M, Cin, Cout, y, stats_partial, nullptr, rows_dev, wrow, seg_grp, sign_src, keys, stream);
 }
 
 int papc_mlp_gemm_rows_f32(int a_mode, const float *x, int64_t ldx, const papc_group_src *grp,
diff --git a/papc_amd/csrc/mlp_stream.hip b/papc_amd/csrc/mlp_stream.hip
--- a/papc_amd/csrc/mlp_stream.hip
+++ b/papc_amd/csrc/mlp_stream.hip
@@ -52,10 +52,11 @@
 __device__ __forceinline__ floatx2_t pk_fma(floatx2_t a, floatx2_t b, floatx2_t c) { return __builtin_elementwise_fma(a, b, c); }
 
 template <int AMODE, int EPI, int KB16, int CK, int WN, bool ASM, bool CP = false, int KV = KB16 * 16, bool NR = false, int CBW = WN * 32, bool PS = false, int NWT = 8,
-          bool GS = false>
+          bool GS = false, bool SG = false>
 __global__ __launch_bounds__(NWT * 64, NWT / 4) void stream_kernel(GemmArgs p, StreamGeo geo)
 {
     static_assert(!GS || EPI == EPI_STORE_GMAX || EPI == EPI_GMAX, "GS: group-max epilogues only");
+    static_assert(!SG || (EPI == EPI_STORE && AMODE == A_BNRELU && ASM && !CP && !NR && KV == KB16 * 16 && NWT == 8), "SG: the storing BN+ReLU forward of a compacted stack only");
     static_assert(NWT == 8 || NWT == 12, "two or three waves per SIMD");
     static_assert(!PS || (CP && AMODE == A_DY_MAX), "PS: the compacted max-layer dX only (the one flavour where the result is bit-identical)");
     static_assert(!CP || ((AMODE == A_DY_DENSE || AMODE == A_DY_MAX) && EPI == EPI_STORE_RED && ASM && PAPC_STREAM_PK), "CP: dX flavours of the asm ring only");
@@ -459,7 +460,7 @@
         rsc[wn] = rsh[wn] = rmu[wn] = ris[wn] = 0.f;
         if (EPI == EPI_STORE_RED) { rsc[wn] = p.rd.scale[col]; rsh[wn] = p.rd.shift[col]; rmu[wn] = p.rd.mean[col]; ris[wn] = p.rd.invstd[col]; }
         gmx[wn] = -INFINITY; gmn[wn] = INFINITY; gix[wn] = 0; gin[wn] = 0;
-        if constexpr (GS) gin[wn] = (p.gm.sgn[col] < 0.f) ? (int)0x80000000u : 0;
+        if constexpr (GS || SG) gin[wn] = (p.gm.sgn[col] < 0.f) ? (int)0x80000000u : 0;
     }
 
     auto epilogue = [&](int row0, int sub) {
@@ -486,6 +487,14 @@
                 __builtin_amdgcn_sched_barrier(0);
             }
             return;
+        }
+        [[maybe_unused]] int sgv[4] = {0, 0, 0, 0};
+        if constexpr (SG) {
+            typedef int i32x4 __attribute__((ext_vector_type(4)));
+            i32x4 q;
+            const int32_t *sp = p.gm.seg + (row0 >> 3);
+            asm volatile("s_load_dwordx4 %0, %1, 0x0\n\ts_waitcnt lgkmcnt(0)" : "=s"(q) : "s"(sp));
+            sgv[0] = q[0]; sgv[1] = q[1]; sgv[2] = q[2]; sgv[3] = q[3];
         }
 #pragma unroll
         for (int wn = 0; wn < WN; ++wn) {
@@ -510,6 +519,8 @@
                 }
                 }
             } else {
+                [[maybe_unused]] float bk = -INFINITY;
+                [[maybe_unused]] int bo = 0;
 #pragma unroll
                 for (int r = 0; r < 16; ++r) {
                     const int ro = (r & 3) + 8 * (r >> 2);
@@ -517,6 +528,25 @@
                     if (EPI != EPI_GMAX && cok) yp[(int64_t)ro * ldy] = v;
                     s1[wn] += v;
                     s2[wn] = fmaf(v, v, s2[wn]);
+                    if constexpr (SG) {
+                        const float key = __int_as_float(__float_as_int(v) ^ gin[wn]);
+                        if (key > bk) { bk = key; bo = ro; }
+                        if ((r & 3) == 3 && ((r >> 2) == 3 || sgv[((r >> 2) + 1) & 3] != sgv[r >> 2])) {
+                            float vmx = bk;
+                            int imx = row0 + 4 * hi + bo;
+                            const float omx = __shfl_xor(vmx, 32);
+                            const int oix = __shfl_xor(imx, 32);
+                            if (omx > vmx || (omx == vmx && oix < imx)) { vmx = omx; imx = oix; }
+                            if (hi == 0) {
+                                unsigned u = __float_as_uint(vmx);
+                                u = (u == 0x80000000u) ? 0u : u;
+                                u = (u & 0x80000000u) ? ~u : (u | 0x80000000u);
+                                const unsigned long long k = ((unsigned long long)u << 32) | (unsigned)~imx;
+                                __hip_atomic_fetch_max(p.gm.keys + (int64_t)sgv[r >> 2] * p.Nout + col, k, __ATOMIC_RELAXED, __HIP_MEMORY_SCOPE_AGENT);
+                            }
+                            bk = -INFINITY; bo = ro;
+                        }
+                    }
                     if (GM) {
                         const int off = sub * 32 + ro + 4 * hi;
                         if constexpr (GS) {
@@ -710,9 +740,10 @@
     return ncu;
 }
 
-template <int AMODE, int EPI, int KB16, int WN, bool CP = false, int KV = KB16 * 16, bool NR = false, int CBW = WN * 32, bool PS = false>
+template <int AMODE, int EPI, int KB16, int WN, bool CP = false, int KV = KB16 * 16, bool NR = false, int CBW = WN * 32, bool PS = false, bool SG = false>
 static int stream_go(const GemmArgs &p, const StreamGeo &geo, hipStream_t st)
 {
+    static_assert(!SG || (!CP && !PS), "SG: a forward flavour");
     constexpr bool KR = (KV != KB16 * 16);
     constexpr int KBF = KR ? KB16 - 1 : KB16;
     constexpr int CK2 = (KBF == 6) ? 1 : 2;
@@ -736,6 +767,12 @@
         const int rc = check_launch("mlp stream gemm (compacted)");
         return rc ? rc : 1;
     }
+    if constexpr (SG) {
+        if (!knob(KNOB_STREAM_ASM)) return 0;
+        hipLaunchKernelGGL((stream_kernel<AMODE, EPI, KB16, CK, WN, true, false, KV, NR, CBW, false, 8, false, true>), grid, dim3(512), 0, st, p, geo);
+        const int rc = check_launch("mlp stream gemm (ragged group keys)");
+        return rc ? rc : 1;
+    }
     if constexpr (AMODE == A_XYZ) hipLaunchKernelGGL((stream_kernel<AMODE, EPI, KB16, CK, WN, false>), grid, dim3(512), 0, st, p, geo);
     else if (knob(KNOB_STREAM_ASM)) {
         if constexpr ((EPI == EPI_XYZ_RED || (EPI == EPI_STORE_RED && AMODE == A_DY_MAX && KB16 == 16)) && WN == 2 && !NR && KV == KB16 * 16) {
@@ -838,6 +875,11 @@
         geo.kgshift = s;
     }
     geo.n_units = (int)((p.M / 32) >> geo.ushift);
+    if (p.gm.keys) {
+        if (!(amode == A_BNRELU && epi == EPI_STORE && geo.rows_dev && p.gm.seg && p.gm.sgn)) return why(13);
+        if (p.Kin == 128 && p.Nout % 128 == 0) return stream_go<A_BNRELU, EPI_STORE, 8, 4, false, 128, false, 128, false, true>(p, geo, st);
+        return why(14);
+    }
     if (amode == A_BNRELU && epi == EPI_STORE) return stream_pick<A_BNRELU, EPI_STORE>(p, geo, st);
     if (amode == A_BNRELU && epi == EPI_GMAX) return knob(KNOB_STREAM_ASM) ? stream_pick<A_BNRELU, EPI_GMAX>(p, geo, st) : 0;
     if (amode == A_BNRELU && epi == EPI_STORE_GMAX) return stream_pick<A_BNRELU, EPI_STORE_GMAX>(p, geo, st);
diff --git a/papc_amd/csrc/sa_mlp.hip b/papc_amd/csrc/sa_mlp.hip
--- a/papc_amd/csrc/sa_mlp.hip
+++ b/papc_amd/csrc/sa_mlp.hip
@@ -17,6 +17,9 @@
 int pfn_bwd_sparse_impl(const float *features, const int32_t *num_voxels, const int32_t *coors, int P, int T, float vx, float vy, float x_offset, float y_offset,
                         const float *w, int C, const float *gout, const int32_t *argmax, const float *mean, const float *invstd, const float *scale,
                         const float *shift, float *partial, int zero_padded, papc_stream_t stream);
+int bn_finalize_clear(const float *stats_partial, int n_tiles, int64_t M, int C, const float *gamma, const float *beta, float eps, float momentum,
+                      float *mean, float *invstd, float *scale, float *shift, float *running_mean, float *running_var, void *clr, int64_t bytes,
+                      hipStream_t st);
 int pfn_bwd_fold_finalize(const float *partial, int n_chunks, float *sums, int64_t M, const float *w, int C, const double *gram, const float *mean,
                           const float *invstd, const float *scale, float *dgamma, float *dbeta, float *dw, int flags, unsigned *ticket, hipStream_t st);
 
@@ -48,6 +51,7 @@
     int32_t *gbuf_i;
     float *P, *wfeat;
     double *gpart;
+    unsigned long long *keys;
 };
 struct BwdPtrs {
     float *c12[PAPC_SA_MAX_LAYERS];
@@ -73,6 +77,11 @@
 }
 static bool defer_room(const papc_sa_grads &gr, int n) { return gr.defer && gr.defer->jobs && gr.defer->count + n <= gr.defer->capacity; }
 static inline int cin_of(const papc_sa_plan &p, int l) { return l == 0 ? p.cin0 : p.d.cout[l - 1]; }
+static inline bool seg_epi_widths(const papc_sa_plan &p)
+{
+    const int L = p.d.n_layers;
+    return p.compact && p.d.pool && L >= 2 && cin_of(p, L - 1) == 128 && p.d.cout[L - 1] % 128 == 0;
+}
 
 static int dw_rows_per_chunk(int64_t M, int cout, int cin, int min_rows = 256)
 {
@@ -131,6 +140,7 @@
     if (p.gmax) f.gbuf_i = c.take<int32_t>(2 * (size_t)G * p.d.cout[L - 1]);
     if (p.lin0) f.wfeat = c.take<float>((size_t)p.d.cout[0] * p.d.D);
     if (p.xyz1) f.gpart = c.take<double>((size_t)papc_xyz_parts(M) * 16 + 16);
+    if (seg_epi_widths(p)) f.keys = c.take<unsigned long long>((size_t)G * p.d.cout[L - 1]);
     return c.off;
 }
 
@@ -515,6 +525,7 @@
     int cmax = 0;
     for (int l = 0; l < L; ++l) cmax = std::max(cmax, d.cout[l]);
     const size_t stats_stride = (size_t)(std::max(parts, p.lin0 ? papc_lingather_parts(M) : 0) + R_c) * 2 * cmax;
+    const bool seg_epi = seg_epi_widths(p) && !ev && knob(KNOB_SEG_EPI) && papc_mlp_seg_epi_ok(M, cin_of(p, L - 1), d.cout[L - 1]);
 
     const float *prev_y = nullptr, *prev_sc = nullptr, *prev_sh = nullptr;
     int cin = p.cin0;
@@ -567,6 +578,9 @@
             SA_CALL(papc_lingather_fwd_f32(s.P, &grp, d.B, ly.w, cin, d.xyz_first ? 0 : d.D, ly.b, cout, y, stats, st));
         } else if (l == 0) {
             SA_CALL(papc_mlp_gemm_f32(A_GROUP_, nullptr, 0, &grp, nullptr, nullptr, ly.w, ly.b, M, cin, cout, y, stats, gm_ref, st));
+        } else if (p.compact && seg_epi && l == L - 1) {
+            SA_CALL(papc_mlp_gemm_rows_keys_f32(prev_y, cin, prev_sc, prev_sh, ly.w, ly.b, M, cin, cout, y, stats, io->compact->rows,
+                                                wstats ? io->compact->wrow : nullptr, io->compact->seg_grp, ly.gamma, f.keys, st));
         } else if (p.compact) {
             SA_CALL(papc_mlp_gemm_rows_w_f32(A_BNRELU_, prev_y, cin, nullptr, prev_sc, prev_sh, ly.w, ly.b, M, cin, cout, y, stats, nullptr, io->compact->rows,
                                              wstats ? io->compact->wrow : nullptr, st));
@@ -578,12 +592,17 @@
             parts_l += R_c;
         }
         if (ev) SA_CALL(papc_bn_eval_consts_f32(ly.running_mean, ly.running_var, ly.gamma, ly.beta, d.eps, cout, cst, cst + cout, cst + 2 * cout, cst + 3 * cout, st));
+        else if (seg_epi && l == L - 2)
+            SA_CALL(bn_finalize_clear(stats, parts_l, M, cout, ly.gamma, ly.beta, d.eps, d.momentum, cst, cst + cout, cst + 2 * cout, cst + 3 * cout,
+                                      ly.running_mean, ly.running_var, f.keys, (int64_t)G * d.cout[L - 1] * 8, as_stream(st)));
         else SA_CALL(papc_bn_finalize_f32(stats, parts_l, M, cout, ly.gamma, ly.beta, d.eps, d.momentum, cst, cst + cout, cst + 2 * cout, cst + 3 * cout,
                                           ly.running_mean, ly.running_var, st));
         prev_y = y; prev_sc = cst + 2 * cout; prev_sh = cst + 3 * cout;
         cin = cout;
     }
     if (!d.pool) return papc_bn_relu_f32(prev_y, prev_sc, prev_sh, M, cin, io->out, st);
+    if (p.compact && seg_epi)
+        return papc_bn_relu_select_seg_f32(f.keys, prev_y, cin, io->compact->start, io->layer[L - 1].gamma, prev_sc, prev_sh, (int)G, io->out, s.argmax, s.gbuf_f, st);
     if (p.compact) return papc_bn_relu_max_seg_f32(prev_y, cin, io->compact->start, prev_sc, prev_sh, (int)G, io->out, s.argmax, s.gbuf_f, st);
     if (p.gmax) return papc_bn_select_max_f32(s.gbuf_f, s.gbuf_f + G * cin, f.gbuf_i, f.gbuf_i + G * cin, prev_sc, prev_sh, G, cin, io->out, s.argmax, st);
     return papc_bn_relu_max_f32(prev_y, prev_sc, prev_sh, G, d.K, cin, io->out, s.argmax, st);
```

After: 22140 (median of 6 runs). 1.01x the previous value.
